# mayuelala/FollowYourClick

Hardware: AMD Instinct MI355X
Metric: denoised frames/sec, 16f x 512^2 clip @ 25 DDIM steps (higher is better)
Workload: dtype bf16; 1 GPU; configs[1]: AnimationPipeline DDIM loop, SD-1.5 UNet3D + mm_sd_v15-shaped motion modules (random init), 1 clip/GPU of 16 frames 512x512, 25 DDIM steps, CFG 8.0, mask + first-frame concat, fps/flow conditioning; frames=16, height=512, width=512, ddim_steps=25, parallelism=dp1 (independent clips, weight broadcast 0.00 GiB in 0.00s)

## Files before the change

### followyourclick_amd/_build.py

```python
import concurrent.futures as cf
import hashlib
import os
import shutil
import subprocess
import sys

HERE = os.path.dirname(os.path.abspath(__file__))
CSRC = os.path.join(HERE, "csrc")
EXTRA = os.environ.get("FYC_BUILD_EXTRA", "").split()
LIB = os.path.abspath(os.environ.get("FYC_BUILD_LIB") or os.path.join(HERE, "libfyc_hip.so"))
OBJ = os.path.join(HERE, "_obj") if not (EXTRA or os.environ.get("FYC_BUILD_LIB")) else LIB + ".obj"
SOURCES = ["api.hip", "gemm.hip", "gemm_bf16_plain.hip", "gemm_bf16_conv.hip", "gemm_bf16_act.hip", "gemm_f16_plain.hip", "gemm_f16_conv.hip", "gemm_f16_act.hip", "gemm_f32.hip", "gemm_bf16_t3.hip", "gemm_f16_t3.hip", "gemm_f32_t3.hip", "gemm_f32x3.hip", "gemm_f32x3_t3.hip", "attention.hip", "attention_small.hip", "attention_medium.hip", "attention_large.hip", "attention_small_f16.hip", "attention_medium_f16.hip", "attention_large_f16.hip", "attention_f32x3.hip", "attention_wide.hip", "attention_wide_f16.hip", "attention_wide_f32x3.hip", "temporal_attn.hip", "temporal_attn_f32x3.hip", "temporal_block.hip", "temporal_block_rr.hip", "ff_block.hip", "panel_linear.hip", "norm.hip", "elementwise.hip"]
FLAGS = ["--offload-arch=gfx950", "-O3", "-std=c++17", "-fPIC", "-ffp-contract=off", "-Wno-unused-value",
         "-mllvm", "-amdgpu-mfma-vgpr-form=1"]
AGPR_SOURCES = {"ff_block.hip", "panel_linear.hip", "temporal_block_rr.hip", "attention_wide.hip", "attention_wide_f16.hip", "attention_wide_f32x3.hip"}


NO_SLP_SOURCES = set(filter(None, os.environ.get("FYC_NO_SLP", "ff_block.hip,gemm_f32x3.hip,gemm_f32x3_t3.hip").split(",")))


NO_NAN_SOURCES = {s for s in SOURCES if s.startswith("attention")}


def _flags(src: str):
    fl = FLAGS
    if src in AGPR_SOURCES:
        fl = [f for f in FLAGS if f not in ("-mllvm", "-amdgpu-mfma-vgpr-form=1")]
    if src in NO_SLP_SOURCES:
        fl = fl + ["-fno-slp-vectorize"]
    if src in NO_NAN_SOURCES and os.environ.get("FYC_ATTN_HONOR_NANS") != "1":
        fl = fl + ["-fno-honor-nans"]
    return fl + EXTRA


def _hipcc() -> str:
    for c in (os.environ.get("HIPCC"), shutil.which("hipcc"), "/opt/rocm/bin/hipcc"):
        if c and os.path.exists(c):
            return c
    raise RuntimeError("hipcc not found (need ROCm with gfx950 support)")


def _digest(path: str) -> str:
    h = hashlib.sha256()
    headers = sorted(os.path.join(CSRC, f) for f in os.listdir(CSRC) if f.endswith(".h"))
    for dep in [path, *headers, os.path.join(HERE, "..", "include", "fyc.h")]:
        with open(dep, "rb") as f:
            h.update(f.read())
    h.update(" ".join(_flags(os.path.basename(path))).encode())
    return h.hexdigest()


def source_digest() -> str:
    h = hashlib.sha256()
    files = sorted(f for f in os.listdir(CSRC) if f.endswith((".hip", ".h")))
    for f in files:
        h.update(f.encode())
        with open(os.path.join(CSRC, f), "rb") as fh:
            h.update(fh.read())
    with open(os.path.join(HERE, "..", "include", "fyc.h"), "rb") as fh:
        h.update(fh.read())
    for src in SOURCES:
        h.update((src + " " + " ".join(_flags(src))).encode())
    return h.hexdigest()


def family_digest(family: str = "gemm") -> str:
    if family != "gemm":
        raise ValueError(family)
    h = hashlib.sha256()
    files = sorted(f for f in os.listdir(CSRC) if f.startswith("gemm") and f.endswith((".hip", ".h"))) + ["fyc_common.h"]
    for f in files:
        h.update(f.encode())
        with open(os.path.join(CSRC, f), "rb") as fh:
            h.update(fh.read())
    for src in SOURCES:
        if src.startswith("gemm"):
            h.update((src + " " + " ".join(_flags(src))).encode())
    return h.hexdigest()


def _compile(src: str) -> str:
    path = os.path.join(CSRC, src)
    obj = os.path.join(OBJ, src.replace(".hip", ".o"))
    stamp = obj + ".sha"
    dig = _digest(path)
    if os.path.exists(obj) and os.path.exists(stamp) and open(stamp).read() == dig:
        return obj
    cmd = [_hipcc(), *_flags(src), "-c", path, "-o", obj]
    r = subprocess.run(cmd, capture_output=True, text=True)
    if r.returncode != 0:
        raise RuntimeError(f"hipcc failed for {src}:\n{r.stderr[-4000:]}")
    with open(stamp, "w") as f:
        f.write(dig)
    return obj

# ... 21 lines not shown
```

### followyourclick_amd/_lib.py

```python
from __future__ import annotations

import ctypes as C
import os

HERE = os.path.dirname(os.path.abspath(__file__))
LIB_PATH = os.environ.get("FYC_LIB_PATH") or os.path.join(HERE, "libfyc_hip.so")

FYC_F32, FYC_BF16, FYC_F16 = 0, 1, 2
GEMM_PLAIN, GEMM_CONV3X3, GEMM_CONV3X3_UP2, GEMM_CONV_T3 = 0, 1, 2, 3
EPI_LINEAR, EPI_GEGLU, EPI_HEADS = 0, 1, 2
ACT_NONE, ACT_GELU, ACT_QUICK_GELU = 0, 1, 2
PRODUCTS_EXACT, PRODUCTS_SPLIT_BF16 = 0, 1

i32, i64, f32, vp = C.c_int32, C.c_int64, C.c_float, C.c_void_p


class GemmArgs(C.Structure):
    _fields_ = [("a", vp), ("a2", vp), ("w", vp), ("bias", vp), ("rowbias", vp), ("residual", vp), ("out", vp),
                ("seg_out", vp * 3), ("seg_transposed", i32 * 3), ("seg_ld", i32 * 3),
                ("M", i32), ("N", i32), ("K", i32),
                ("lda", i32), ("ldw", i32), ("ldo", i32), ("ldr", i32), ("ldrb", i32), ("k_split", i32), ("lda2", i32),
                ("stride_a", i64), ("stride_w", i64), ("stride_o", i64),
                ("batch", i32), ("mode", i32), ("epilogue", i32),
                ("Hout", i32), ("Wout", i32), ("Hin", i32), ("Win", i32), ("Cin", i32), ("conv_stride", i32), ("conv_pad", i32),
                ("rows_per_batch", i32), ("seg_cols", i32), ("heads", i32), ("tokens", i32),
                ("out_scale", f32), ("dtype", i32), ("tile", i32), ("act", i32), ("ln_stats", vp), ("ln_colsum", vp),
                ("ln_nparts", i32), ("ln_eps", f32), ("chan_parts", vp), ("cs_rows", i32), ("row_parts", vp), ("row_nparts", i32), ("workspace", vp), ("workspace_bytes", i64),
                ("t3_frames", i32), ("t3_rows", i32), ("f32_products", i32)]


class AttnArgs(C.Structure):
    _fields_ = [("q", vp), ("k", vp), ("vt", vp), ("o", vp),
                ("batch", i32), ("heads", i32), ("n_q", i32), ("n_k", i32), ("d", i32),
                ("ldo", i32), ("ldvt", i32), ("kv_batch_div", i32), ("o_accumulate", i32),
                ("scale", f32), ("o_scale", f32), ("dtype", i32), ("q_batch_mod", i32), ("f32_products", i32)]


class AttnMaskArgs(C.Structure):
    _fields_ = [("attn", AttnArgs), ("causal", i32)]


class TAttnArgs(C.Structure):
    _fields_ = [("qkv", vp), ("o", vp), ("clips", i32), ("frames", i32), ("pixels", i32), ("heads", i32), ("d", i32),
                ("scale", f32), ("dtype", i32), ("rope_cos", vp), ("rope_sin", vp), ("f32_products", i32)]


class GnStatsArgs(C.Structure):
    _fields_ = [("x", vp), ("stats", vp), ("rows", i32), ("C", i32), ("groups", i32), ("rows_per_sample", i32), ("dtype", i32),
                ("pad_", i32), ("workspace", vp), ("workspace_bytes", i64)]


class GnApplyArgs(C.Structure):
    _fields_ = [("x", vp), ("stats", vp), ("gamma", vp), ("beta", vp), ("y", vp),
                ("rows", i32), ("C", i32), ("groups", i32), ("rows_per_sample", i32), ("eps", f32), ("silu", i32), ("dtype", i32)]


class ChanStatsReduceArgs(C.Structure):
    _fields_ = [("parts", vp), ("cs", vp), ("rows", i32), ("N", i32), ("cs_rows", i32), ("tile_rows", i32), ("slots", i32), ("out_rows", i32)]


class GnApplyCsArgs(C.Structure):
    _fields_ = [("x1", vp), ("cs1", vp), ("x2", vp), ("cs2", vp), ("gamma", vp), ("beta", vp), ("y", vp),
                ("C1", i32), ("C2", i32), ("rows", i32), ("groups", i32), ("rows_per_sample", i32), ("eps", f32), ("silu", i32),
                ("dtype", i32), ("cs_rows", i32), ("parts1", vp), ("parts2", vp),
                ("tile_rows1", i32), ("slots1", i32), ("tile_rows2", i32), ("slots2", i32), ("parts_cs_rows", i32)]


class LayerNormArgs(C.Structure):
    _fields_ = [("x", vp), ("gamma", vp), ("beta", vp), ("pe", vp), ("y", vp),
                ("rows", i32), ("C", i32), ("eps", f32), ("pe_div", i32), ("pe_rows", i32), ("dtype", i32)]


class RowStatsArgs(C.Structure):
    _fields_ = [("x", vp), ("stats", vp), ("rows", i32), ("C", i32), ("eps", f32), ("dtype", i32)]


class SoftmaxArgs(C.Structure):
    _fields_ = [("x", vp), ("rows", i64), ("cols", i32), ("ld", i32), ("dtype", i32), ("causal_rows", i32)]


class ConcatArgs(C.Structure):
    _fields_ = [("a", vp), ("b", vp), ("y", vp), ("rows", i64), ("c1", i32), ("c2", i32), ("dtype", i32)]


class RepeatArgs(C.Structure):
    _fields_ = [("src", vp), ("dst", vp), ("bytes", i64), ("times", i32)]


class SiluArgs(C.Structure):
    _fields_ = [("x", vp), ("y", vp), ("n", i64)]


class CastArgs(C.Structure):
    _fields_ = [("x", vp), ("y", vp), ("rows", i64), ("cols", i32), ("ld", i32), ("dtype", i32)]


class UnetInputArgs(C.Structure):
    _fields_ = [("latents", vp), ("mask", vp), ("first", vp), ("x", vp),
                ("B", i32), ("F", i32), ("HW", i32), ("c_latent", i32), ("c_pad", i32), ("cfg_dup", i32), ("mask_frames", i32),
                ("dtype", i32), ("mode", i32)]


class CfgDdimArgs(C.Structure):
    _fields_ = [("pred", vp), ("latents", vp), ("coef", vp),
                ("B", i32), ("F", i32), ("HW", i32), ("c_latent", i32), ("ld", i32), ("cfg", i32), ("guidance", f32),
                ("pred_type", i32), ("clip_sample", i32), ("dtype", i32), ("pred_single", vp), ("video_scale", f32),
                ("variance_noise", vp), ("sigma", f32), ("clipped_model_output", i32)]


class CfgDdimRescaleArgs(C.Structure):
    _fields_ = [("step", CfgDdimArgs), ("guidance_rescale", f32), ("workspace", vp), ("workspace_bytes", i64)]


class CfgSolverArgs(C.Structure):
    _fields_ = [("pred", vp), ("latents", vp), ("coef", vp),
                ("B", i32), ("F", i32), ("HW", i32), ("c_latent", i32), ("ld", i32), ("cfg", i32), ("guidance", f32),
                ("dtype", i32), ("pred_single", vp), ("video_scale", f32),
                ("hist_out", vp), ("hist_1", vp), ("hist_2", vp), ("order", i32),
                ("guidance_rescale", f32), ("workspace", vp), ("workspace_bytes", i64)]


class NchwInArgs(C.Structure):
    _fields_ = [("z", vp), ("x", vp), ("N", i32), ("C", i32), ("HW", i32), ("c_pad", i32), ("scale", f32), ("dtype", i32)]


class NhwcOutArgs(C.Structure):
    _fields_ = [("x", vp), ("y", vp), ("N", i32), ("C", i32), ("HW", i32), ("ld", i32),
                ("mul", f32), ("add", f32), ("lo", f32), ("hi", f32), ("dtype", i32)]


class EmbedArgs(C.Structure):
    _fields_ = [("ids", vp), ("table", vp), ("pos", vp), ("out", vp), ("rows", i64), ("seq", i32), ("C", i32), ("vocab", i32),
                ("dtype", i32)]


class PatchifyArgs(C.Structure):
    _fields_ = [("image", vp), ("out", vp), ("B", i32), ("Cin", i32), ("H", i32), ("W", i32), ("P", i32), ("ld", i32), ("dtype", i32)]


class TemporalBlockArgs(C.Structure):
    _fields_ = [("x", vp), ("out", vp), ("w_qkv", vp), ("colsum", vp), ("bias", vp), ("pe_bias", vp), ("w_out", vp), ("b_out", vp),
                ("clips", i32), ("frames", i32), ("pixels", i32), ("heads", i32), ("d", i32), ("C", i32),
                ("scale", C.c_float), ("eps", C.c_float), ("dtype", i32), ("wstream", vp)]


class FFBlockArgs(C.Structure):
    _fields_ = [("x", vp), ("residual", vp), ("out", vp), ("wstream", vp), ("b_out", vp), ("chan_parts", vp), ("cs_rows", i32),
                ("rows", i32), ("C", i32), ("hidden", i32), ("eps", C.c_float), ("dtype", i32)]


class PanelLinearArgs(C.Structure):
    _fields_ = [("x", vp), ("residual", vp), ("out", vp), ("wstream", vp), ("bias", vp), ("gn_cs", vp), ("gn_gamma", vp), ("gn_beta", vp),
                ("gn_rows_per_sample", i32), ("gn_stat_samples", i32), ("gn_groups", i32), ("gn_eps", C.c_float),
                ("rows", i32), ("N", i32), ("K", i32), ("dtype", i32), ("gn_parts", vp), ("gn_tile_rows", i32), ("gn_slots", i32)]


class PackConv3x3Args(C.Structure):
    _fields_ = [("w", vp), ("out", vp), ("O", i32), ("I", i32), ("dtype", i32)]


class PackGegluArgs(C.Structure):
    _fields_ = [("w", vp), ("b", vp), ("w_out", vp), ("b_out", vp), ("O", i32), ("I", i32), ("dtype", i32)]


OPS = {
    "fyc_gemm": GemmArgs, "fyc_attention": AttnArgs, "fyc_attention_masked": AttnMaskArgs, "fyc_temporal_attention": TAttnArgs,
    "fyc_gn_stats": GnStatsArgs, "fyc_gn_apply": GnApplyArgs, "fyc_layernorm": LayerNormArgs,
    "fyc_softmax_rows": SoftmaxArgs, "fyc_concat_channels": ConcatArgs, "fyc_silu_f32": SiluArgs,
    "fyc_cast_from_f32": CastArgs, "fyc_cast_to_f32": CastArgs, "fyc_unet_input": UnetInputArgs,
    "fyc_cfg_ddim_step": CfgDdimArgs, "fyc_cfg_ddim_step_rescaled": CfgDdimRescaleArgs, "fyc_cfg_solver_step": CfgSolverArgs, "fyc_nchw_to_nhwc": NchwInArgs, "fyc_nhwc_to_nchw": NhwcOutArgs,
    "fyc_embed_tokens": EmbedArgs, "fyc_patchify": PatchifyArgs, "fyc_row_stats": RowStatsArgs,
    "fyc_gn_apply_cs": GnApplyCsArgs, "fyc_chan_stats_reduce": ChanStatsReduceArgs,
    "fyc_pack_conv3x3": PackConv3x3Args, "fyc_pack_geglu": PackGegluArgs, "fyc_temporal_block": TemporalBlockArgs,
    "fyc_ff_block": FFBlockArgs, "fyc_panel_linear": PanelLinearArgs, "fyc_repeat": RepeatArgs,
}
MISC = ["fyc_version", "fyc_last_error", "fyc_init", "fyc_device_caps", "fyc_set_tuning", "fyc_gemm_row_parts", "fyc_gemm_stat_layout", "fyc_gemm_workspace_bytes", "fyc_gn_stats_workspace", "fyc_temporal_block_supported", "fyc_temporal_block_wstream_bytes",
        "fyc_ff_block_supported", "fyc_ff_block_wstream_bytes", "fyc_panel_linear_supported", "fyc_panel_linear_wstream_bytes",
        "fyc_cfg_ddim_rescale_workspace_bytes", "fyc_cfg_solver_workspace_bytes"]

_lib = None
FYC_VERSION = 308


class FycError(RuntimeError):
    pass


def load() -> C.CDLL:
    global _lib
    if _lib is not None:
        return _lib
    if not os.path.exists(LIB_PATH):
        raise FycError(f"{LIB_PATH} is missing: build it with `python -m followyourclick_amd._build` "
                       "(hipcc --offload-arch=gfx950). There is no CPU fallback.")
    lib = C.CDLL(LIB_PATH)
    lib.fyc_version.restype = C.c_int
    ab_build = bool(os.environ.get("FYC_LIB_PATH"))
    if lib.fyc_version() != FYC_VERSION and not ab_build:
        raise FycError(f"{LIB_PATH} reports ABI version {lib.fyc_version()}, this binding was written against {FYC_VERSION}: argument structs differ "
                       "between major versions - rebuild the library (`python -m followyourclick_amd._build`)")
    lib.fyc_last_error.restype = C.c_char_p
    lib.fyc_init.argtypes = [vp]
    lib.fyc_device_caps.argtypes = [C.POINTER(i64)]
    lib.fyc_set_tuning.argtypes = [C.c_int, C.c_int]
    if not ab_build or hasattr(lib, "fyc_gemm_row_parts"):
        lib.fyc_gemm_row_parts.argtypes = [C.POINTER(GemmArgs)]
        lib.fyc_gemm_row_parts.restype = C.c_int
        lib.fyc_gemm_stat_layout.argtypes = [C.POINTER(GemmArgs), C.POINTER(i32), C.POINTER(i32)]
        lib.fyc_gemm_stat_layout.restype = C.c_int
        lib.fyc_gemm_workspace_bytes.argtypes = [C.POINTER(GemmArgs)]
        lib.fyc_gemm_workspace_bytes.restype = i64
    if not ab_build or hasattr(lib, "fyc_gn_stats_workspace"):
        lib.fyc_gn_stats_workspace.argtypes = [C.POINTER(GnStatsArgs)]
        lib.fyc_gn_stats_workspace.restype = i64
    if not ab_build or hasattr(lib, "fyc_temporal_block_supported"):
        lib.fyc_temporal_block_supported.argtypes = [C.POINTER(TemporalBlockArgs)]
        lib.fyc_temporal_block_supported.restype = C.c_int
    if not ab_build or hasattr(lib, "fyc_temporal_block_wstream_bytes"):
        lib.fyc_temporal_block_wstream_bytes.argtypes = []
        lib.fyc_temporal_block_wstream_bytes.restype = i64
    if not ab_build or hasattr(lib, "fyc_ff_block_supported"):
        lib.fyc_ff_block_supported.argtypes = [C.POINTER(FFBlockArgs)]
        lib.fyc_ff_block_supported.restype = C.c_int
        lib.fyc_ff_block_wstream_bytes.argtypes = []
        lib.fyc_ff_block_wstream_bytes.restype = i64
    if not ab_build or hasattr(lib, "fyc_panel_linear_supported"):
        lib.fyc_panel_linear_supported.argtypes = [C.POINTER(PanelLinearArgs)]
        lib.fyc_panel_linear_supported.restype = C.c_int
        lib.fyc_panel_linear_wstream_bytes.argtypes = [i32, i32]
        lib.fyc_panel_linear_wstream_bytes.restype = i64
    if not ab_build or hasattr(lib, "fyc_cfg_ddim_rescale_workspace_bytes"):
        lib.fyc_cfg_ddim_rescale_workspace_bytes.argtypes = [C.POINTER(CfgDdimRescaleArgs)]
        lib.fyc_cfg_ddim_rescale_workspace_bytes.restype = i64
    if not ab_build or hasattr(lib, "fyc_cfg_solver_workspace_bytes"):
        lib.fyc_cfg_solver_workspace_bytes.argtypes = [C.POINTER(CfgSolverArgs)]
        lib.fyc_cfg_solver_workspace_bytes.restype = i64
    for name, st in OPS.items():
        if ab_build and not hasattr(lib, name):
            continue
        fn = getattr(lib, name)
        fn.argtypes = [C.POINTER(st), vp]
        fn.restype = C.c_int
    _lib = lib
    return lib


def check(rc: int, what: str) -> None:
    if rc != 0:
        raise FycError(f"{what} failed (rc={rc}): {load().fyc_last_error().decode(errors='replace')}")
```

### followyourclick_amd/csrc/gemm_kernel.h

```cpp
#pragma once
#include <mutex>
#include <type_traits>

#include "fyc_common.h"

namespace fycg {

constexpr int FYC_MAX_DEVICES = 64;

struct GemmP {
  const char* a; const char* a2; const char* w; const float* bias; const float* rowbias; const char* residual; char* out;
  char* seg_out[3]; int seg_transposed[3]; int seg_ld[3];
  int M, N, K, lda, ldw, ldo, ldr, ldrb, k_split, lda2;
  long long stride_a, stride_w, stride_o;
  int mode, epilogue;
  int Hout, Wout, Hin, Win, Cin, conv_stride, conv_pad;
  int rows_per_batch, seg_cols, heads, tokens, head_dim;
  float out_scale;
  int act;
  const float* ln_stats; const float* ln_colsum;
  int ln_nparts; float ln_eps;
  float* chan_parts; int cs_rows, cs_slots;
  float* row_parts; int row_nparts;
  int tiles_m, tiles_n;
  int strip;
  int up_exact2; float up_sh, up_sw;
  int colc;
  int rb_tile;
  int rb_slots;
  int splitk; int t3_frames; float* ws;
  int stagger;
  int wide;
  const char* zero;
  int res_acc;
  float inv_seg_cols, inv_head_dim;
  int fast1;
  int heads_pk;
  int pre;
  int phase_delay; int t3_rows;
  unsigned long long* trace;
};
static_assert(sizeof(GemmP) == 392, "GemmP grew: the kernel-argument offsets of every instantiation move");

#ifdef FYC_TRACE
#define FYC_STAMP_DECL int fyc_trace_n = 0
#define FYC_STAMP(p, wave, lane)                                                                                         \
  do {                                                                                                                   \
    if ((p).trace != nullptr && ((wave) & 3) == 0 && (lane) == 0 && fyc_trace_n < 128)                                   \
      (p).trace[((size_t)blockIdx.x * 2 + ((wave) >> 2)) * 128 + fyc_trace_n] = __builtin_amdgcn_s_memtime();            \
    ++fyc_trace_n;                                                                                                       \
  } while (0)
#define FYC_STAMP_E(p, wave, lane, cnt)                                                                                  \
  do {                                                                                                                   \
    if ((p).trace != nullptr && ((wave) & 3) == 0 && (lane) == 0 && (cnt) < 128)                                         \
      (p).trace[65536 + ((size_t)blockIdx.x * 2 + ((wave) >> 2)) * 128 + (cnt)] = __builtin_amdgcn_s_memtime();          \
    ++(cnt);                                                                                                             \
  } while (0)
#else
#define FYC_STAMP_DECL
#define FYC_STAMP(p, wave, lane) do { } while (0)
#define FYC_STAMP_E(p, wave, lane, cnt) do { } while (0)
#endif

__device__ __forceinline__ void tile_coords(const GemmP& p, int t, int& tile_m, int& tile_n) {
  if (p.strip <= 0) { tile_n = t % p.tiles_n; tile_m = t / p.tiles_n; return; }
  const int per_strip = p.strip * p.tiles_m;
  const int s = t / per_strip, r = t - s * per_strip;
  const int n0 = s * p.strip;
  const int w = min(p.strip, p.tiles_n - n0);
  tile_m = r / w;
  tile_n = n0 + r - tile_m * w;
}

template <typename T> struct Mma;
template <> struct Mma<bf16_t> {
  typedef bf16x8 Frag;
  __device__ static __forceinline__ f32x4 mma(Frag a, Frag b, f32x4 c) {
    return __builtin_amdgcn_mfma_f32_16x16x32_bf16(a, b, c, 0, 0, 0);
  }
};
template <> struct Mma<f16_t> {
  typedef f16x8 Frag;
  __device__ static __forceinline__ f32x4 mma(Frag a, Frag b, f32x4 c) {
    return __builtin_amdgcn_mfma_f32_16x16x32_f16(a, b, c, 0, 0, 0);
  }
};
template <> struct Mma<float> {
  typedef f32x4 Frag;
  __device__ static __forceinline__ f32x4 mma(Frag a, Frag b, f32x4 c) {
    c = __builtin_amdgcn_mfma_f32_16x16x4f32(a[0], b[0], c, 0, 0, 0);
    c = __builtin_amdgcn_mfma_f32_16x16x4f32(a[1], b[1], c, 0, 0, 0);
// ... 195 lines not shown
#pragma unroll
  for (int i = 1; i < WTM; ++i) rb_same = rb_same && rbo[i] == rbo[0];
  const bool has_ln = LN && p.ln_stats != nullptr;
  auto pass1_fast = [&](auto ln_c, auto rb_c) __attribute__((always_inline)) {
    constexpr bool HAS_LN = decltype(ln_c)::value, HAS_RB = decltype(rb_c)::value;
    f32x2 rs2[WTM], nm2[WTM];
#pragma unroll
    for (int i = 0; i < WTM; ++i) { rs2[i] = (f32x2){rs[i], rs[i]}; nm2[i] = (f32x2){-rs[i] * mu[i], -rs[i] * mu[i]}; }
    const float* rb0 = HAS_RB ? rbc + rbo[0] : colc;
    f32x4 b4n = *reinterpret_cast<const f32x4*>(colc + nl_w0 + g * 4), s4n = (f32x4){0.f, 0.f, 0.f, 0.f}, r4n = (f32x4){0.f, 0.f, 0.f, 0.f};
    if (HAS_LN) s4n = *reinterpret_cast<const f32x4*>(colc + BN + nl_w0 + g * 4);
    if (HAS_RB) r4n = *reinterpret_cast<const f32x4*>(rb0 + nl_w0 + g * 4);
#pragma unroll
    for (int j = 0; j < WTN; ++j) {
      const int nl = nl_w0 + j * 16 + g * 4;
      f32x4 b4 = b4n;
      const f32x4 s4 = s4n;
      if (HAS_RB) { b4[0] += r4n[0]; b4[1] += r4n[1]; b4[2] += r4n[2]; b4[3] += r4n[3]; }
      __builtin_amdgcn_sched_barrier(0);
      if (j + 1 < WTN) {
        b4n = *reinterpret_cast<const f32x4*>(colc + nl + 16);
        if (HAS_LN) s4n = *reinterpret_cast<const f32x4*>(colc + BN + nl + 16);
        if (HAS_RB) r4n = *reinterpret_cast<const f32x4*>(rb0 + nl + 16);
      }
      const f32x2 b01 = {b4[0], b4[1]}, b23 = {b4[2], b4[3]}, s01 = {s4[0], s4[1]}, s23 = {s4[2], s4[3]};
#pragma unroll
      for (int i = 0; i < WTM; ++i) {
        f32x2 v01 = {acc[i][j][0], acc[i][j][1]}, v23 = {acc[i][j][2], acc[i][j][3]};
        if (HAS_LN) {
          v01 = __builtin_elementwise_fma(v01, rs2[i], __builtin_elementwise_fma(nm2[i], s01, b01));
          v23 = __builtin_elementwise_fma(v23, rs2[i], __builtin_elementwise_fma(nm2[i], s23, b23));
        } else {
          v01 = v01 + b01; v23 = v23 + b23;
        }
        unsigned lo = Pair16<T>::pack(v01[0], v01[1]), hi = Pair16<T>::pack(v23[0], v23[1]);
        asm volatile("" : "+v"(lo), "+v"(hi));
        pk[i][j] = (u32x2){lo, hi};
      }
      __builtin_amdgcn_sched_barrier(0);
    }
  };
  if (p.out_scale == 1.0f && (rbc == nullptr || rb_same) && p.fast1) {
    if (has_ln) { if (rbc != nullptr) pass1_fast(std::true_type{}, std::true_type{}); else pass1_fast(std::true_type{}, std::false_type{}); }
    else { if (rbc != nullptr) pass1_fast(std::false_type{}, std::true_type{}); else pass1_fast(std::false_type{}, std::false_type{}); }
  } else {
  f32x4 b4n = *reinterpret_cast<const f32x4*>(colc + nl_w0 + g * 4), s4n = (f32x4){0.f, 0.f, 0.f, 0.f};
  if (LN && p.ln_stats) s4n = *reinterpret_cast<const f32x4*>(colc + BN + nl_w0 + g * 4);
#pragma unroll
  for (int j = 0; j < WTN; ++j) {
    const int nl = nl_w0 + j * 16 + g * 4;
    const f32x4 b4 = b4n, s4 = s4n;
    __builtin_amdgcn_sched_barrier(0);
    if (j + 1 < WTN) {
      b4n = *reinterpret_cast<const f32x4*>(colc + nl + 16);
      if (LN && p.ln_stats) s4n = *reinterpret_cast<const f32x4*>(colc + BN + nl + 16);
    }
#pragma unroll
    for (int i = 0; i < WTM; ++i) {
      f32x4 v = acc[i][j];
      if (LN && p.ln_stats) {
#pragma unroll
        for (int r = 0; r < 4; ++r) v[r] = rs[i] * (v[r] - mu[i] * s4[r]);
      }
#pragma unroll
      for (int r = 0; r < 4; ++r) v[r] += b4[r];
      if (rbc != nullptr) {
        const f32x4 r4 = *reinterpret_cast<const f32x4*>(rbc + rbo[i] + nl);
#pragma unroll
        for (int r = 0; r < 4; ++r) v[r] += r4[r];
      }
      unsigned lo = Pair16<T>::pack(v[0] * p.out_scale, v[1] * p.out_scale), hi = Pair16<T>::pack(v[2] * p.out_scale, v[3] * p.out_scale);
      asm volatile("" : "+v"(lo), "+v"(hi));
      pk[i][j] = (u32x2){lo, hi};
    }
    __builtin_amdgcn_sched_barrier(0);
  }
  }
  FYC_STAMP_E(p, wave, lane, ecnt);
  const int lrow = lane / CPR, lch = lane - lrow * CPR;
  const bool lact = lrow < RPP;
  const int n_lane = n_w0 + lch * 8;
  const int first_sample = do_cs ? (tile_m * BM) / p.cs_rows : 0;
  const bool one_slot = p.cs_slots == 1;
  float cs8[8], cq8[8];
#pragma unroll
  for (int e = 0; e < 8; ++e) cs8[e] = cq8[e] = 0.f;
  int cur_slot = one_slot ? 0 : -1;
  auto flush_tree = [&](int slot) __attribute__((always_inline)) {
    float* red = reinterpret_cast<float*>(stg);
    float* own = cacc + (wm + slot) * (BN * 2);
    constexpr int NCOL = CPR * 8, ROWS_LIVE = RPP < 16 ? RPP : 16;
#pragma unroll
    for (int ph = 0; ph < 2; ++ph) {
      if (lact) {
        const float* src = ph ? cq8 : cs8;
        *reinterpret_cast<f32x4*>(red + lane * 8) = (f32x4){src[0], src[1], src[2], src[3]};
        *reinterpret_cast<f32x4*>(red + lane * 8 + 4) = (f32x4){src[4], src[5], src[6], src[7]};
      }
      asm volatile("s_waitcnt lgkmcnt(0)" ::: "memory");
#pragma unroll 1
      for (int c = lane; c < NCOL; c += 64) {
        float t = 0.f;
#pragma unroll
        for (int r = 0; r < ROWS_LIVE; ++r) t += red[r * NCOL + c];
        own[(nl_w0 + c) * 2 + ph] = t;
      }
      asm volatile("s_waitcnt lgkmcnt(0)" ::: "memory");
    }
#pragma unroll
    for (int e = 0; e < 8; ++e) cs8[e] = cq8[e] = 0.f;
  };
#pragma unroll
  for (int i = 0; i < WTM; ++i) {
    if (do_cs && !one_slot) {
      const int slot = (tile_m * BM + (wm * WTM + i) * 16) / p.cs_rows - first_sample;
      if (slot != cur_slot) { if (cur_slot >= 0) flush_tree(cur_slot); cur_slot = slot; }
    }
#pragma unroll
    for (int j = 0; j < WTN; ++j) *reinterpret_cast<u32x2*>(stg + r16 * PITCH + j * 32 + g * 8) = pk[i][j];
    asm volatile("s_waitcnt lgkmcnt(0)" ::: "memory");
#pragma unroll
    for (int q = 0; q < NQ; ++q) {
      u32x4 v4q;
      {
        const int rowc = (q * RPP + lrow) < 15 ? (q * RPP + lrow) : 15;
        v4q = *reinterpret_cast<const u32x4*>(stg + rowc * PITCH + lch * 16);
      }
      asm volatile("s_waitcnt lgkmcnt(0)" ::: "memory");
      const int row = q * RPP + lrow;
      const int m = tile_m * BM + (wm * WTM + i) * 16 + row;
      float rsum = 0.f, rsq = 0.f;
      const bool live = lact && row < 16 && m < p.M && n_lane < p.N;
      if (live) {
        const u32x4 v4 = v4q;
        *reinterpret_cast<u32x4*>(O + (long long)m * p.ldo + n_lane) = v4;
        if (do_cs || do_rp) {
#pragma unroll
          for (int e = 0; e < 4; ++e) {
            const float x0 = Pair16<T>::lo(v4[e]), x1 = Pair16<T>::hi(v4[e]);
            if (do_cs) {
              cs8[2 * e] += x0; cq8[2 * e] = __builtin_fmaf(x0, x0, cq8[2 * e]);
              cs8[2 * e + 1] += x1; cq8[2 * e + 1] = __builtin_fmaf(x1, x1, cq8[2 * e + 1]);
            }
            if (do_rp) { rsum += x0 + x1; rsq = __builtin_fmaf(x0, x0, __builtin_fmaf(x1, x1, rsq)); }
          }
        }
      }
      if (do_rp && live) {
        float* dst = racc + ((wm * WTM + i) * 16 + row) * 2;
        lds_add(dst, rsum); lds_add(dst + 1, rsq);
      }
    }
    asm volatile("s_waitcnt lgkmcnt(0)" ::: "memory");
  }
  FYC_STAMP_E(p, wave, lane, ecnt);
  if (do_cs) flush_tree(cur_slot);
  if (do_cs || do_rp) stats_flush<BM, BN, WGM, WGM * WGN * 64>(p, cacc, tile_m, tile_n, wave * 64 + lane);
}

template <typename T, int BM, int BN, int WGM, int WGN, int STG_BYTES, int MODE>
__device__ __forceinline__ void epilogue_heads_packed(const GemmP& p, f32x4 (&acc)[BM / WGM / 16][BN / WGN / 16], int tile_m, int tile_n,
                                                      char* stg_stage, int wave, int lane, const char* pre) {
  static_assert(sizeof(T) == 2, "16-bit outputs only (bf16 / f16)");
  constexpr int WTM = BM / WGM / 16, WTN = BN / WGN / 16;
  constexpr bool LN = (MODE == FYC_GEMM_PLAIN);
  constexpr int PITCH = WTN * 32 + 16, CPR = WTN * 2, RPP = 64 / CPR, NQ = (16 + RPP - 1) / RPP;
  constexpr int SLICE = 16 * PITCH;
  static_assert(WGM * WGN * SLICE + 2 * BN * 4 <= STG_BYTES, "staging + column constants must fit in one ring stage");
  const int wm = wave / WGN, wn = wave % WGN;
  const int g = lane >> 4, r16 = lane & 15;
  __builtin_amdgcn_s_barrier();
  char* stg = stg_stage + wave * SLICE;
  float* colc = reinterpret_cast<float*>(stg_stage + WGM * WGN * SLICE);
  if (pre != nullptr) colc = reinterpret_cast<float*>(const_cast<char*>(pre) + BM * 8);
  else stage_col_constants<BN, LN>(p, colc, tile_m * BM, tile_n, wave * 64 + lane);
  const bool has_ln = LN && p.ln_stats != nullptr;
  f32x2 rs2[WTM], nm2[WTM];
#pragma unroll
  for (int i = 0; i < WTM; ++i) {
    float mu = 0.f, rs = 1.f;
    if (has_ln) {
      if (pre != nullptr) pre_ln_row<BM>(pre, (wm * WTM + i) * 16 + r16, mu, rs);
      else if (tile_m * BM + (wm * WTM + i) * 16 + r16 < p.M) ln_row(p, tile_m * BM + (wm * WTM + i) * 16 + r16, mu, rs);
    }
    rs2[i] = (f32x2){rs * p.out_scale, rs * p.out_scale}; nm2[i] = (f32x2){-rs * mu, -rs * mu};
  }
  const int nl_w0 = wn * WTN * 16, n_w0 = tile_n * BN + nl_w0;
  const f32x2 sc2 = {p.out_scale, p.out_scale};
  u32x2 pk[WTM][WTN];
  auto pass1 = [&](auto ln_c) __attribute__((always_inline)) {
    constexpr bool HAS_LN = decltype(ln_c)::value;
#pragma unroll
    for (int j = 0; j < WTN; ++j) {
      const int nl = nl_w0 + j * 16 + g * 4;
      const f32x4 b4 = *reinterpret_cast<const f32x4*>(colc + nl);
      f32x4 s4 = (f32x4){0.f, 0.f, 0.f, 0.f};
      if (HAS_LN) s4 = *reinterpret_cast<const f32x4*>(colc + BN + nl);
      __builtin_amdgcn_sched_barrier(0);
      const f32x2 b01 = {b4[0], b4[1]}, b23 = {b4[2], b4[3]}, s01 = {s4[0], s4[1]}, s23 = {s4[2], s4[3]};
#pragma unroll
      for (int i = 0; i < WTM; ++i) {
        f32x2 v01 = {acc[i][j][0], acc[i][j][1]}, v23 = {acc[i][j][2], acc[i][j][3]};
        if (HAS_LN) {
          v01 = __builtin_elementwise_fma(v01, rs2[i], sc2 * __builtin_elementwise_fma(nm2[i], s01, b01));
          v23 = __builtin_elementwise_fma(v23, rs2[i], sc2 * __builtin_elementwise_fma(nm2[i], s23, b23));
        } else {
          v01 = (v01 + b01) * sc2; v23 = (v23 + b23) * sc2;
        }
        unsigned lo = Pair16<T>::pack(v01[0], v01[1]), hi = Pair16<T>::pack(v23[0], v23[1]);
        asm volatile("" : "+v"(lo), "+v"(hi));
        pk[i][j] = (u32x2){lo, hi};
      }
      __builtin_amdgcn_sched_barrier(0);
    }
  };
  if (has_ln) pass1(std::true_type{}); else pass1(std::false_type{});
  const int lrow = lane / CPR, lch = lane - lrow * CPR;
  const int n_a = n_w0 + lch * 8;
// ... 114 lines not shown
        unsigned lo = Pair16<T>::pack(lo2.x, lo2.y), hi = Pair16<T>::pack(hi2.x, hi2.y);
        asm volatile("" : "+v"(lo), "+v"(hi));
        pk[i][jo] = (u32x2){lo, hi};
      }
      __builtin_amdgcn_sched_barrier(0);
    }
  };
  if (has_ln) pass1(std::true_type{}); else pass1(std::false_type{});
  const int lrow = lane / CPR, lch = lane - lrow * CPR;
  const bool lact = lrow < RPP;
  const int n_out = p.N >> 1;
  const int n_lane = ((tile_n * BN + nl_w0) >> 1) + lch * 8;
#pragma unroll
  for (int i = 0; i < WTM; ++i) {
#pragma unroll
    for (int jo = 0; jo < OT; ++jo) *reinterpret_cast<u32x2*>(stg + r16 * PITCH + jo * 32 + g * 8) = pk[i][jo];
    asm volatile("s_waitcnt lgkmcnt(0)" ::: "memory");
    u32x4 v4q[NQ];
#pragma unroll
    for (int q = 0; q < NQ; ++q) {
      const int rowc = (q * RPP + lrow) < 15 ? (q * RPP + lrow) : 15;
      v4q[q] = *reinterpret_cast<const u32x4*>(stg + rowc * PITCH + lch * 16);
    }
    asm volatile("s_waitcnt lgkmcnt(0)" ::: "memory");
#pragma unroll
    for (int q = 0; q < NQ; ++q) {
      const int row = q * RPP + lrow;
      const int m = tile_m * BM + (wm * WTM + i) * 16 + row;
      if (lact && row < 16 && m < p.M && n_lane < n_out) *reinterpret_cast<u32x4*>(O + (long long)m * p.ldo + n_lane) = v4q[q];
    }
  }
}

template <typename T, int BM, int BN, int WGM, int WGN>
__device__ __forceinline__ void load_residual_acc(const GemmP& p, f32x4 (&acc)[BM / WGM / 16][BN / WGN / 16], int tile_m, int tile_n, int wave, int lane) {
  constexpr int WTM = BM / WGM / 16, WTN = BN / WGN / 16;
  const int wm = wave / WGN, wn = wave % WGN;
  const int g = lane >> 4, r16 = lane & 15;
  const T* R = reinterpret_cast<const T*>(p.residual);
  const T* zero = reinterpret_cast<const T*>(p.zero);
  constexpr int NP = WTN / 2;
  u32x4 raw16[WTM][NP > 0 ? NP : 1];
  u32x2 raw[WTM][WTN - 2 * NP > 0 ? WTN - 2 * NP : 1];
#pragma unroll
  for (int i = 0; i < WTM; ++i) {
    const int m = tile_m * BM + (wm * WTM + i) * 16 + r16;
#pragma unroll
    for (int jp = 0; jp < NP; ++jp) {
      const int n = tile_n * BN + (wn * WTN + 2 * jp) * 16 + g * 8;
      const T* ptr = (m < p.M && n < p.N) ? R + ((long long)m * p.ldr + n) : zero;
      raw16[i][jp] = *reinterpret_cast<const u32x4*>(ptr);
    }
#pragma unroll
    for (int j = 2 * NP; j < WTN; ++j) {
      const int n = tile_n * BN + (wn * WTN + j) * 16 + g * 4;
      const T* ptr = (m < p.M && n < p.N) ? R + ((long long)m * p.ldr + n) : zero;
      raw[i][j - 2 * NP] = *reinterpret_cast<const u32x2*>(ptr);
    }
  }
  __builtin_amdgcn_sched_barrier(0);
#pragma unroll
  for (int i = 0; i < WTM; ++i) {
#pragma unroll
    for (int jp = 0; jp < NP; ++jp) {
      unsigned x0 = raw16[i][jp][0], x1 = raw16[i][jp][1], y0 = raw16[i][jp][2], y1 = raw16[i][jp][3];
      auto a = __builtin_amdgcn_permlane16_swap(x0, y0, false, false);
      auto b = __builtin_amdgcn_permlane16_swap(x1, y1, false, false);
      auto c = __builtin_amdgcn_permlane32_swap(a[0], a[1], false, false);
      auto d = __builtin_amdgcn_permlane32_swap(b[0], b[1], false, false);
      acc[i][2 * jp] = (f32x4){Pair16<T>::lo(c[0]), Pair16<T>::hi(c[0]), Pair16<T>::lo(d[0]), Pair16<T>::hi(d[0])};
      acc[i][2 * jp + 1] = (f32x4){Pair16<T>::lo(c[1]), Pair16<T>::hi(c[1]), Pair16<T>::lo(d[1]), Pair16<T>::hi(d[1])};
    }
#pragma unroll
    for (int j = 2 * NP; j < WTN; ++j)
      acc[i][j] = (f32x4){Pair16<T>::lo(raw[i][j - 2 * NP][0]), Pair16<T>::hi(raw[i][j - 2 * NP][0]), Pair16<T>::lo(raw[i][j - 2 * NP][1]), Pair16<T>::hi(raw[i][j - 2 * NP][1])};
  }
}

template <typename T, int BM, int BN, int WGM, int WGN, int EPI, int STG_BYTES, int MODE, bool WIDE>
__device__ __forceinline__ void gemm_epilogue(const GemmP& p, f32x4 (&acc)[BM / WGM / 16][BN / WGN / 16], int tile_m, int tile_n,
                                              long long bz, char* stg_stage, int wave, int lane, const char* pre, int& ecnt) {
  constexpr int WTM = BM / WGM / 16, WTN = BN / WGN / 16;
  constexpr bool LN = (MODE == FYC_GEMM_PLAIN);
  const int wm = wave / WGN, wn = wave % WGN;
  const int g = lane >> 4, r16 = lane & 15;
  T* O = reinterpret_cast<T*>(p.out) + bz * p.stride_o;
  const T* R = reinterpret_cast<const T*>(p.residual);
  if constexpr (WIDE && EPI == FYC_EPI_HEADS && sizeof(T) == 2) {
    if (p.fast1 && p.heads_pk) {
      epilogue_heads_packed<T, BM, BN, WGM, WGN, STG_BYTES, MODE>(p, acc, tile_m, tile_n, stg_stage, wave, lane, pre);
      return;
    }
  }
  if constexpr (WIDE && EPI == FYC_EPI_HEADS) {
    constexpr int JG = (WTN + 1) / 2;
    constexpr int PITCH = JG * 64 + 16;
    static_assert(WGM * WGN * 16 * PITCH + 2 * BN * 4 <= STG_BYTES, "staging + column constants must fit in one ring stage");
    __builtin_amdgcn_s_barrier();
    char* stg = stg_stage + wave * (16 * PITCH);
    float* colc = reinterpret_cast<float*>(stg_stage + WGM * WGN * 16 * PITCH);
    if (pre != nullptr) colc = reinterpret_cast<float*>(const_cast<char*>(pre) + BM * 8);
    else stage_col_constants<BN, LN>(p, colc, tile_m * BM, tile_n, wave * 64 + lane);
    const int n_w0 = tile_n * BN + wn * WTN * 16, nl_w0 = wn * WTN * 16;
#pragma unroll
    for (int i = 0; i < WTM; ++i) {
      const int m0 = tile_m * BM + (wm * WTM + i) * 16;
      float ln_mu = 0.f, ln_rs = 1.f;
      if (LN && p.ln_stats) {
        if (pre != nullptr) pre_ln_row<BM>(pre, (wm * WTM + i) * 16 + r16, ln_mu, ln_rs);
        else if (m0 + r16 < p.M) ln_row(p, m0 + r16, ln_mu, ln_rs);
      }
      const int b = m0 / p.tokens, tok0 = m0 - b * p.tokens;
#pragma unroll
      for (int h = 0; h < 2; ++h) {
        const int j0 = h * JG;
        const int nj = (WTN - j0 < JG) ? (WTN - j0) : JG;
        if (nj <= 0) continue;
#pragma unroll
        for (int jj = 0; jj < JG; ++jj) {
          const int jo = j0 + jj;
          if (jo >= WTN) continue;
          const int nl = nl_w0 + jo * 16 + g * 4;
          f32x4 v = acc[i][jo];
          const f32x4 s4 = *reinterpret_cast<const f32x4*>(colc + BN + nl), b4 = *reinterpret_cast<const f32x4*>(colc + nl);
#pragma unroll
          for (int r = 0; r < 4; ++r) v[r] = ((LN && p.ln_stats ? ln_rs * (v[r] - ln_mu * s4[r]) : v[r]) + b4[r]) * p.out_scale;
          *reinterpret_cast<f32x4*>(stg + r16 * PITCH + (jj * 16 + g * 4) * 4) = v;
        }
        asm volatile("s_waitcnt lgkmcnt(0)" ::: "memory");
        const int n0 = n_w0 + j0 * 16;
        if (m0 < p.M) {
          const int cpr = nj * 2;
          for (int c = lane; c < 16 * cpr; c += 64) {
            const int row = c / cpr, ch = c - row * cpr;
            const int n = n0 + ch * 8;
            if (n >= p.N) continue;
            const int seg = fdiv_small(n, p.inv_seg_cols), cs = n - seg * p.seg_cols;
            if (p.seg_transposed[seg]) continue;
            const int hh = fdiv_small(cs, p.inv_head_dim), di = cs - hh * p.head_dim;
            float v8[8];
            *reinterpret_cast<f32x4*>(v8) = *reinterpret_cast<const f32x4*>(stg + row * PITCH + ch * 32);
            *reinterpret_cast<f32x4*>(v8 + 4) = *reinterpret_cast<const f32x4*>(stg + row * PITCH + ch * 32 + 16);
            T* S = reinterpret_cast<T*>(p.seg_out[seg]);
            store8<T>(S + ((long long)(b * p.heads + hh) * p.tokens + tok0 + row) * p.head_dim + di, v8);
          }
          for (int u = lane; u < nj * 32; u += 64) {
            const int col = u >> 1, half = u & 1;
            const int n = n0 + col;
            if (n >= p.N) continue;
            const int seg = fdiv_small(n, p.inv_seg_cols), cs = n - seg * p.seg_cols;
            if (!p.seg_transposed[seg]) continue;
            const int hh = fdiv_small(cs, p.inv_head_dim), di = cs - hh * p.head_dim;
            float v8[8];
#pragma unroll
            for (int r = 0; r < 8; ++r) v8[r] = *reinterpret_cast<const float*>(stg + (half * 8 + r) * PITCH + col * 4);
            T* S = reinterpret_cast<T*>(p.seg_out[seg]);
            store8<T>(S + ((long long)(b * p.heads + hh) * p.head_dim + di) * p.seg_ld[seg] + tok0 + half * 8, v8);
          }
        }
        asm volatile("s_waitcnt lgkmcnt(0)" ::: "memory");
      }
    }
    return;
  }
  if constexpr (WIDE && EPI == FYC_EPI_LINEAR) {
    epilogue_linear_packed<T, BM, BN, WGM, WGN, STG_BYTES, MODE>(p, acc, tile_m, tile_n, bz, stg_stage, wave, lane, pre, ecnt);
// ... 240 lines not shown
        } else {
          const int seg = n / p.seg_cols, c = n - seg * p.seg_cols;
          const int h = c / p.head_dim, di = c - h * p.head_dim;
          const int b = m / p.tokens, tok = m - b * p.tokens;
          T* S = reinterpret_cast<T*>(p.seg_out[seg]);
#pragma unroll
          for (int r = 0; r < 4; ++r) v[r] *= p.out_scale;
          if (!p.seg_transposed[seg]) {
            ElemIO<T>::st4(S + ((long long)(b * p.heads + h) * p.tokens + tok) * p.head_dim + di, v);
          } else {
#pragma unroll
            for (int r = 0; r < 4; ++r)
              ElemIO<T>::st(S + ((long long)(b * p.heads + h) * p.head_dim + di + r) * p.seg_ld[seg] + tok, v[r]);
          }
        }
      }
      if (do_rp) { float* dst = racc + ((wm * WTM + i) * 16 + r16) * 2; lds_add(dst, st_rs); lds_add(dst + 1, st_rq); }
    }
    }
    if constexpr (STATS_OK) {
      if (do_cs) {
        float* own = cacc + (wm + st_slot) * (BN * 2) + ((wn * WTN) * 16 + g * 4) * 2;
#pragma unroll
        for (int j = 0; j < WTN; ++j) {
#pragma unroll
          for (int r = 0; r < 4; ++r) {
            float sx = xs[j][r], sq = xs[j][r] * xs[j][r];
#pragma unroll
            for (int o = 1; o < 16; o <<= 1) { sx += __shfl_xor(sx, o); sq += __shfl_xor(sq, o); }
            if (r16 == 0) { own[(j * 16 + r) * 2] += sx; own[(j * 16 + r) * 2 + 1] += sq; }
          }
        }
      }
    }
  }
  if (do_cs || do_rp) stats_flush<BM, BN, WGM, WGM * WGN * 64>(p, cacc, tile_m, tile_n, wave * 64 + lane);
  }
}

template <int S> using KStep = std::integral_constant<int, S>;
template <typename T, int BM, int BN, int WGM, int WGN, int MODE, int EPI, int NS, int RB = 128, bool WIDE = false, typename P = T>
__global__ void __launch_bounds__(WGM* WGN * 64) fyc_gemm_kernel(const GemmP p) {
  typedef Mma<P> Tr;
  typedef typename Tr::Frag Frag;
  constexpr int NT = WGM * WGN * 64;
  constexpr int CH = 16 / (int)sizeof(T);
  constexpr int CPR = RB / 16;
  constexpr int BK = CPR * CH;
  constexpr int KSTEPS = RB / 64;
  constexpr int A_IT = BM * CPR / NT, B_IT = BN * CPR / NT;
  constexpr int LOADS = A_IT + B_IT;
  constexpr int WTM = BM / WGM / 16, WTN = BN / WGN / 16;
  static_assert(EPI != FYC_EPI_GEGLU || WTN % 2 == 0, "GEGLU pairs value / gate column blocks inside a wave");
  constexpr bool SPLIT3 = std::is_same<P, f32x3_t>::value;
  static_assert(std::is_same<P, T>::value || (SPLIT3 && std::is_same<T, float>::value && RB == 128 && WGM * WGN == 4),
                "f32x3: float storage, one 32-float K tile per matrix instruction, the 4-wave tiles of the f32 mode");
  constexpr int A_BYTES = BM * RB, STAGE = (BM + BN) * RB;
  constexpr bool STAGGER = (WGM * WGN == 8) && KSTEPS >= 2 && NS == 2;
  static_assert(A_IT * NT == BM * CPR && B_IT * NT == BN * CPR, "tile/threads mismatch");
  static_assert(NS >= 2 && NS <= 4 && (NS - 2) * LOADS < 64, "ring depth");
  extern __shared__ __attribute__((aligned(16))) char smem[];

  const int tid = threadIdx.x, lane = tid & 63;
  const int wave = __builtin_amdgcn_readfirstlane(tid >> 6);
  const int wm = wave / WGN, wn = wave % WGN;

  const int ntiles = p.tiles_m * p.tiles_n;
  auto remap = [&](int t) {
    const int q = ntiles >> 3, r = ntiles & 7, xcd = t & 7, idx = t >> 3;
    return (xcd < r ? xcd * (q + 1) : r * (q + 1) + (xcd - r) * q) + idx;
  };
  const long long bz = blockIdx.z;
  const T* __restrict__ A = reinterpret_cast<const T*>(p.a) + bz * p.stride_a;
  const T* __restrict__ W = reinterpret_cast<const T*>(p.w) + bz * p.stride_w;
  const T* __restrict__ A2 = reinterpret_cast<const T*>(p.a2);
  const T* zero = reinterpret_cast<const T*>(p.zero);

  const int lrow = tid / CPR;
  const int koff = ((tid % CPR) ^ swz_key<RB>(lrow)) * CH;
  constexpr int ROWS_IT = NT / CPR;
  static_assert(ROWS_IT % 16 == 0, "row stride per DMA instruction must keep the swizzle key");
  int i_tm = 0, i_tn = 0;
  unsigned a_base = 0, a2_base = 0, b_base = 0;
  constexpr bool C3 = (MODE == FYC_GEMM_CONV3X3);
  constexpr bool T3 = (MODE == FYC_GEMM_CONV_T3);
  constexpr int TAPS = T3 ? 3 : 9;
  static_assert(!T3 || A_IT * 3 <= 32, "CONV_T3: the presence masks of a thread's rows share one register");
  int a_pos[C3 ? A_IT : 1], a_msk[C3 ? A_IT : 1];
  unsigned t_msk = 0, t_step = 0;
  int a_pix[MODE == FYC_GEMM_CONV3X3_UP2 ? A_IT : 1], a_yx[MODE == FYC_GEMM_CONV3X3_UP2 ? A_IT : 1];
  int tap = 0, c0 = 0;
  const int KT = (p.K + BK - 1) / BK;
  const int S = p.splitk > 1 ? p.splitk : 1;
  auto kt_begin = [&](int work) { return (int)(((long long)(work % S) * KT) / S); };
  auto kt_end = [&](int work) { return (int)(((long long)(work % S + 1) * KT) / S); };
  auto setup_issue = [&](int work) {
    const int t = remap(work / S);
    tile_coords(p, t, i_tm, i_tn);
    const int kt0 = kt_begin(work);
    tap = kt0 % TAPS; c0 = (kt0 / TAPS) * BK;
    if (MODE == FYC_GEMM_PLAIN || S == 1) { tap = 0; c0 = 0; }
    b_base = (unsigned)(i_tn * BN + lrow) * (unsigned)p.ldw + koff;
    if (MODE == FYC_GEMM_PLAIN) {
      a_base = (unsigned)(i_tm * BM + lrow) * (unsigned)p.lda + koff;
      a2_base = (unsigned)(i_tm * BM + lrow) * (unsigned)p.lda2 + koff - p.k_split;
    } else if constexpr (T3) {
      a_base = (unsigned)(i_tm * BM + lrow) * (unsigned)p.Cin + koff;
      t_step = (unsigned)p.t3_rows * (unsigned)p.Cin;
      t_msk = 0;
#pragma unroll
      for (int it = 0; it < A_IT; ++it) {
        const int m = i_tm * BM + lrow + it * ROWS_IT;
        const int f = (m / p.t3_rows) % p.t3_frames;
        const unsigned msk = (f > 0 ? 1u : 0u) | 2u | (f + 1 < p.t3_frames ? 4u : 0u);
        if (m < p.M) t_msk |= msk << (3 * it);
      }
    } else {
#pragma unroll
      for (int it = 0; it < A_IT; ++it) {
        const int m = i_tm * BM + lrow + it * ROWS_IT;
        const int hw = p.Hout * p.Wout;
        const int fr = m / hw, rem = m - fr * hw, oy = rem / p.Wout, ox = rem - oy * p.Wout;
        const int iy0 = oy * p.conv_stride - p.conv_pad, ix0 = ox * p.conv_stride - p.conv_pad;
        if (C3) {
          a_pos[it] = fr * p.Hin * p.Win + iy0 * p.Win + ix0;
          int msk = 0;
#pragma unroll
          for (int tp = 0; tp < 9; ++tp) {
            const int iy = iy0 + tp / 3, ix = ix0 + tp % 3;
            if ((unsigned)iy < (unsigned)p.Hin && (unsigned)ix < (unsigned)p.Win) msk |= 1 << tp;
          }
          a_msk[it] = (m < p.M) ? msk : 0;
        } else {
          a_pix[it] = (m < p.M) ? fr * p.Hin * p.Win : -1;
          a_yx[it] = (iy0 << 16) | (ix0 & 0xffff);
        }
      }
    }
  };

  auto src_a = [&](int it, int k0) -> const T* {
    if (MODE == FYC_GEMM_PLAIN) {
      const int m = i_tm * BM + lrow + it * ROWS_IT;
      const int k = k0 + koff;
      if (m >= p.M || k >= p.K) return zero;
      if (A2 != nullptr && k >= p.k_split) return A2 + (size_t)(a2_base + (unsigned)(it * ROWS_IT) * (unsigned)p.lda2 + k0);
      return A + (size_t)(a_base + (unsigned)(it * ROWS_IT) * (unsigned)p.lda + k0);
    } else if constexpr (T3) {
      const unsigned e = a_base + (unsigned)(it * ROWS_IT) * (unsigned)p.Cin + (unsigned)(tap - 1) * t_step + (unsigned)c0;
      return ((t_msk >> (3 * it + tap)) & 1u) ? A + (size_t)e : zero;
    } else if (C3) {
      const int ky = tap / 3, kx = tap - 3 * ky;
      const int pos = a_pos[it] + ky * p.Win + kx;
      return ((a_msk[it] >> tap) & 1) ? A + (size_t)((unsigned)pos * (unsigned)p.Cin + (c0 + koff)) : zero;
    } else {
      const int ky = tap / 3, kx = tap - 3 * ky;
      const int iy = (a_yx[it] >> 16) + ky, ix = (int)(short)(a_yx[it] & 0xffff) + kx;
      const bool ok = a_pix[it] >= 0 && (unsigned)iy < (unsigned)p.Hout && (unsigned)ix < (unsigned)p.Wout;
      int sy, sx;
      if (p.up_exact2) { sy = iy >> 1; sx = ix >> 1; }
      else {
        sy = min((int)floorf((float)iy * p.up_sh), p.Hin - 1);
        sx = min((int)floorf((float)ix * p.up_sw), p.Win - 1);
      }
      return ok ? A + (size_t)((unsigned)(a_pix[it] + sy * p.Win + sx) * (unsigned)p.Cin + c0 + koff) : zero;
    }
  };
  auto src_b = [&](int it, int k0) -> const T* {
    const int n = i_tn * BN + lrow + it * ROWS_IT;
    return (n < p.N && k0 + koff < p.K) ? W + (size_t)(b_base + (unsigned)(it * ROWS_IT) * (unsigned)p.ldw + k0) : zero;
  };

  f32x4 acc[WTM][WTN];
  FYC_STAMP_DECL;
  int fyc_trace_e = 0;

  const int g = lane >> 4, r16 = lane & 15;
  const int sw = swz_key<RB>(r16);
  constexpr bool FRAG_ALL = sizeof(T) == 2 && (WTM * WTN + WTM + WTN) * 4 <= 150;
  constexpr bool FRAG_ROW = sizeof(T) == 2 && !FRAG_ALL;
  constexpr int PF = (WTN >= 8) ? 2 : (WTN >= 4 ? 4 : 6);
  auto compute = [&](int stage, auto first, auto end) {
    constexpr int s0 = decltype(first)::value, s1 = decltype(end)::value;
    const char* sA = smem + stage * STAGE + (wm * WTM * 16 + r16) * RB;
    const char* sB = smem + stage * STAGE + A_BYTES + (wn * WTN * 16 + r16) * RB;
#pragma unroll
    for (int s = 0; s < KSTEPS; ++s) {
      if (s < s0 || s >= s1) continue;
      const int coff = ((4 * s + g) ^ sw) * 16;
      if constexpr (FRAG_ROW) {
        constexpr int RING = PF + 1;
        Frag bfr[WTN], ar[RING];
#pragma unroll
        for (int j = 0; j < WTN; ++j) bfr[j] = *reinterpret_cast<const Frag*>(sB + j * 16 * RB + coff);
#pragma unroll
        for (int i = 0; i < PF && i < WTM; ++i) ar[i % RING] = *reinterpret_cast<const Frag*>(sA + i * 16 * RB + coff);
#pragma unroll
        for (int i = 0; i < WTM; ++i) {
          if (i + PF < WTM) ar[(i + PF) % RING] = *reinterpret_cast<const Frag*>(sA + (i + PF) * 16 * RB + coff);
          __builtin_amdgcn_sched_barrier(0);
#pragma unroll
          for (int j = 0; j < WTN; ++j) acc[i][j] = Tr::mma(bfr[j], ar[i % RING], acc[i][j]);
          __builtin_amdgcn_sched_barrier(0);
        }
        continue;
      }
      Frag af[WTM], bf[WTN];
#pragma unroll
      for (int i = 0; i < WTM; ++i) af[i] = *reinterpret_cast<const Frag*>(sA + i * 16 * RB + coff);
#pragma unroll
      for (int j = 0; j < WTN; ++j) bf[j] = *reinterpret_cast<const Frag*>(sB + j * 16 * RB + coff);
      if (FRAG_ALL) __builtin_amdgcn_sched_barrier(0);
#pragma unroll
      for (int i = 0; i < WTM; ++i)
#pragma unroll
        for (int j = 0; j < WTN; ++j) acc[i][j] = Tr::mma(bf[j], af[i], acc[i][j]);
      if (FRAG_ALL) __builtin_amdgcn_sched_barrier(0);
    }
  };
  constexpr bool XSTEP = FRAG_ALL && KSTEPS == 2 && (WTM * WTN + 2 * (WTM + WTN)) * 4 <= 190;
  auto compute_xstep = [&](int stage, auto&& between) {
    const char* sA = smem + stage * STAGE + (wm * WTM * 16 + r16) * RB;
    const char* sB = smem + stage * STAGE + A_BYTES + (wn * WTN * 16 + r16) * RB;
    const int coff0 = (g ^ sw) * 16, coff1 = ((4 + g) ^ sw) * 16;
    Frag af0[WTM], bf0[WTN], af1[WTM], bf1[WTN];
#pragma unroll
    for (int i = 0; i < WTM; ++i) af0[i] = *reinterpret_cast<const Frag*>(sA + i * 16 * RB + coff0);
#pragma unroll
    for (int j = 0; j < WTN; ++j) bf0[j] = *reinterpret_cast<const Frag*>(sB + j * 16 * RB + coff0);
    __builtin_amdgcn_sched_barrier(0);
#pragma unroll
    for (int i = 0; i < WTM; ++i) af1[i] = *reinterpret_cast<const Frag*>(sA + i * 16 * RB + coff1);
#pragma unroll
    for (int j = 0; j < WTN; ++j) bf1[j] = *reinterpret_cast<const Frag*>(sB + j * 16 * RB + coff1);
    __builtin_amdgcn_sched_barrier(0);
// ... 200 lines not shown
  q.tiles_n = (p.N + BN - 1) / BN;
  q.rb_tile = (p.colc && p.rowbias != nullptr && p.rows_per_batch % BM == 0) ? 1 : 0;
  q.rb_slots = (WIDE && EPI == FYC_EPI_LINEAR && p.rowbias != nullptr && !q.rb_tile) ? rowbias_slots(BM, p.rows_per_batch) : 0;
  {
    constexpr int BK = (RB / 16) * (16 / (int)sizeof(T));
    const int kt = (p.K + BK - 1) / BK;
    const bool rb_ok = p.rowbias == nullptr || (EPI == FYC_EPI_LINEAR && (q.rb_tile || q.rb_slots > 0));
    q.pre = (PRE_BUILT && g_fyc_tuning[FYC_TUNE_NO_PRESTAGE] != 1 && kt >= 2 && !(q.splitk > 1) && p.ln_nparts == 0 && rb_ok && p.wide &&
             (p.ln_stats == nullptr || (p.M % 2 == 0 && ((uintptr_t)p.ln_stats % 16) == 0))) ? 1 : 0;
  }
  q.fast1 = g_fyc_tuning[FYC_TUNE_GENERIC_PASS1] == 1 ? 0 : 1;
  q.heads_pk = g_fyc_tuning[FYC_TUNE_HEADS_PACKED] == 1 ? 1 : g_fyc_tuning[FYC_TUNE_HEADS_PACKED] == 2 ? 0 : (p.M <= 8192 ? 1 : 0);
  q.stagger = g_fyc_tuning[FYC_TUNE_NO_STAGGER] == 1 ? 0 : 1;
  q.phase_delay = g_fyc_tuning[FYC_TUNE_PHASE_DELAY] > 0 ? g_fyc_tuning[FYC_TUNE_PHASE_DELAY] : 0;
  q.res_acc = (WIDE && EPI == FYC_EPI_LINEAR && p.residual != nullptr && p.ln_stats == nullptr && !(q.splitk > 1)) ? 1 : 0;
#ifdef FYC_TRACE
  q.trace = g_fyc_trace;
#endif
  q.strip = (q.tiles_n > 4 && g_fyc_tuning[FYC_TUNE_GEMM_STRIP] >= 0) ? (g_fyc_tuning[FYC_TUNE_GEMM_STRIP] > 0 ? g_fyc_tuning[FYC_TUNE_GEMM_STRIP] : (q.tiles_n >= 16 ? 8 : 4)) : 0;
  int occ = (160 * 1024) / smem;
  const int wave_cap = 32 / (WGM * WGN);
  if (occ > wave_cap) occ = wave_cap;
  if (occ < 1) occ = 1;
  long long resident = (long long)n_cu * occ / (batch > 0 ? batch : 1);
  if (resident < n_cu) resident = n_cu;
  const long long ntiles = (long long)q.tiles_m * q.tiles_n * (q.splitk > 1 ? q.splitk : 1);
  dim3 grid((unsigned)(ntiles < resident ? ntiles : resident), 1, batch);
  hipLaunchKernelGGL(kern, grid, dim3(WGM * WGN * 64), smem, st, q);
  FYC_CHECK_LAUNCH("fyc_gemm");
  return 0;
}

template <typename T, int MODE, int EPI, bool WIDE, typename P = T>
int dispatch_cfg(int cfg, int ns, const GemmP& p, int batch, hipStream_t st) {
  if constexpr (!WIDE) {
    if (cfg != 1 && cfg != 2) cfg = (p.N % 128 == 0 || p.N > 512) ? 1 : 2;
    if (cfg == 1) return launch<T, 128, 128, 2, 2, MODE, EPI, 2, 128, false, P>(p, batch, st);
    return launch<T, 128, 64, 2, 2, MODE, EPI, 2, 128, false, P>(p, batch, st);
  } else {
    switch (cfg) {
      case 1: if (ns == 3) return launch<T, 128, 128, 2, 2, MODE, EPI, 3, 128, true>(p, batch, st);
              return launch<T, 128, 128, 2, 2, MODE, EPI, 2, 128, true>(p, batch, st);
      case 2: if constexpr (MODE == FYC_GEMM_PLAIN) {
                if (ns == 4) return launch<T, 128, 64, 2, 2, MODE, EPI, 4, 128, true>(p, batch, st);
                if (ns == 3) return launch<T, 128, 64, 2, 2, MODE, EPI, 3, 128, true>(p, batch, st);
              }
              return launch<T, 128, 64, 2, 2, MODE, EPI, 2, 128, true>(p, batch, st);
      case 3: return launch<T, 256, 128, 4, 2, MODE, EPI, 2, 128, true>(p, batch, st);
      case 4: return launch<T, 256, 64, 4, 1, MODE, EPI, 2, 128, true>(p, batch, st);
      case 5: return launch<T, 256, 320, 4, 2, MODE, EPI, 2, 128, true>(p, batch, st);
      case 6: if constexpr (EPI == FYC_EPI_GEGLU) FYC_FAIL(-2, "fyc_gemm: tile config 6 gives a wave an odd number of column blocks: not built for GEGLU");
              else return launch<T, 128, 320, 2, 4, MODE, EPI, 2, 128, true>(p, batch, st);
      case 7: return launch<T, 256, 256, 2, 4, MODE, EPI, 2, 128, true>(p, batch, st);
      case 8: return launch<T, 128, 320, 2, 2, MODE, EPI, 2, 64, true>(p, batch, st);
      case 10: return launch<T, 128, 128, 2, 2, MODE, EPI, 2, 64, true>(p, batch, st);
      case 11: if constexpr (EPI == FYC_EPI_GEGLU) FYC_FAIL(-2, "fyc_gemm: tile config 11 gives a wave an odd number of column blocks: not built for GEGLU");
               else return launch<T, 128, 160, 2, 2, MODE, EPI, 2, 128, true>(p, batch, st);
    }
    FYC_FAIL(-2, "fyc_gemm: tile config %d not built", cfg);
  }
}

template <typename T, int MODE, int EPI>
int dispatch_ns(int ns, int cfg, const GemmP& p, int batch, hipStream_t st) {
  if constexpr (sizeof(T) == 2) {
    if (p.wide) return dispatch_cfg<T, MODE, EPI, true>(cfg, ns, p, batch, st);
  }
  return dispatch_cfg<T, MODE, EPI, false>(cfg, ns, p, batch, st);
}

int run_bf16_plain(const GemmP& p, int batch, int cfg, int ns, hipStream_t st);
int run_bf16_conv(const GemmP& p, int batch, int cfg, int ns, hipStream_t st);
int run_bf16_act(const GemmP& p, int batch, int cfg, hipStream_t st);
int run_f32(const GemmP& p, int batch, int cfg, hipStream_t st);
constexpr int CFG_F32X3 = 0x100;
int run_f32x3(const GemmP& p, int batch, int cfg, hipStream_t st);
int run_f32x3_t3(const GemmP& p, int batch, int cfg, hipStream_t st);
int run_f16_plain(const GemmP& p, int batch, int cfg, int ns, hipStream_t st);
int run_f16_conv(const GemmP& p, int batch, int cfg, int ns, hipStream_t st);
int run_f16_act(const GemmP& p, int batch, int cfg, hipStream_t st);
int run_bf16_t3(const GemmP& p, int batch, int cfg, int ns, hipStream_t st);
int run_f16_t3(const GemmP& p, int batch, int cfg, int ns, hipStream_t st);
int run_f32_t3(const GemmP& p, int batch, int cfg, hipStream_t st);

}
```

### followyourclick_amd/engine/base.py

```python
from __future__ import annotations

import os
from typing import Optional, Sequence, Tuple

import torch

from .. import _lib as L

Tensor = torch.Tensor

ALLOC_FILL = int(os.environ["FYC_ALLOC_FILL"]) if os.environ.get("FYC_ALLOC_FILL") else None


def empty(*shape, dtype, device) -> Tensor:
    t = torch.empty(*shape, dtype=dtype, device=device)
    if ALLOC_FILL is not None and t.numel():
        t.view(torch.uint8).fill_(ALLOC_FILL)
    return t


def conv_out_size(Hin: int, Win: int, stride: int = 1, pad: int = 1, up2: bool = False, up_size=None) -> Tuple[int, int]:
    if up2:
        return up_size if up_size is not None else (2 * Hin, 2 * Win)
    return (Hin + pad - 2) // stride + 1, (Win + pad - 2) // stride + 1
# ... 21 lines not shown
    sw = os.environ.get("FYC_SIDE_FLASH", "1")
    if sw == "0":
        return False
    if dtype == torch.float32 and getattr(ops, "f32_products", "exact") != "split":
        return False
    can_causal, max_d = getattr(ops, "attention_causal_supported", None), getattr(ops, "attention_max_head_dim", None)
    if can_causal is None or max_d is None or d % 8 or d > max_d() or (d > 160 and d % 32) or (causal and not can_causal()):
        return False
    return sw == "force" or SIDE_FLASH_DEFAULT[family, _DT_WORD[dtype]]


class EngineBase:
    fuse_stats = True
    direct_stats = False

    def new(self, *shape, dtype=None) -> Tensor:
        return empty(*shape, dtype=dtype or self.dtype, device=self.device)

    def zeros(self, *shape, dtype=None) -> Tensor:
        return torch.zeros(*shape, dtype=dtype or self.dtype, device=self.device)

    def _cs_plan(self, rows: int, stat_rows: int, N: int, K: int, mode: int, out_rows: int) -> Optional[ChanStats]:
        if not self.fuse_stats or stat_rows % 16 or rows % stat_rows:
            return None
        if getattr(self.ops, "abi_version", L.FYC_VERSION) < 301 and self.ops.gemm_split_bytes(self.dtype, M=rows, N=N, K=K, mode=mode) > 0:
            return None
        nt, tile_rows, slots = self.ops.gemm_stat_layout(self.dtype, M=rows, N=N, K=K, cs_rows=stat_rows, mode=mode)
        if not 1 <= slots <= 4:
            return None
        return ChanStats(N, out_rows, parts=self.new(nt * slots * N * 2, dtype=torch.float32), tile_rows=tile_rows, slots=slots, rows=rows,
                         stat_rows=stat_rows)

    def _produced(self, st: Optional[ChanStats]) -> Optional[ChanStats]:
        if st is not None and not self.direct_stats:
            self._stats(st)
        return st

    def _stats(self, st: ChanStats) -> Tensor:
        if st.cs is None:
            st.cs = self.new(st.rows // st.out_rows, st.C, 2, dtype=torch.float64)
            self.ops.chan_stats_reduce(st.parts, st.cs, rows=st.rows, N=st.C, cs_rows=st.stat_rows, tile_rows=st.tile_rows, slots=st.slots,
                                       out_rows=st.out_rows)
        return st.cs

    def _direct_limit(self) -> int:
        return 0

    def _direct(self, sts: Sequence[ChanStats], rows_per_sample: int) -> Optional[int]:
        if not self.direct_stats or any(st.parts is None or st.cs is not None for st in sts):
            return None
        srows = sts[0].stat_rows
        if any(st.stat_rows != srows for st in sts) or rows_per_sample % srows:
            return None
        nbytes = 0
        for st in sts:
            tiles = rows_per_sample // st.tile_rows if rows_per_sample % st.tile_rows == 0 else (rows_per_sample - 1) // st.tile_rows + 2
            nbytes += max(tiles, 1) * st.slots * st.C * 8
        return nbytes if nbytes <= self._direct_limit() else None

    def gn_from_stats(self, srcs: Sequence[Tuple[Tensor, Optional[ChanStats]]], gamma: Tensor, beta: Tensor, rows: int,
                      rows_per_sample: int, eps: float, silu: bool, groups: Optional[int] = None) -> Optional[Tensor]:
        sts = [st for _, st in srcs]
        if any(st is None or st.out_rows != sts[0].out_rows for st in sts) or rows_per_sample % sts[0].out_rows:
            return None
        s1 = sts[0]
        kw = {}
        if len(srcs) == 2:
            kw.update(x2=srcs[1][0], C2=sts[1].C)
        if self._direct(sts, rows_per_sample) is not None:
            cs1 = None
            kw.update(parts1=s1.parts, tile_rows1=s1.tile_rows, slots1=s1.slots, parts_cs_rows=s1.stat_rows)
            if len(srcs) == 2:
                kw.update(parts2=sts[1].parts, tile_rows2=sts[1].tile_rows, slots2=sts[1].slots)
        else:
            cs1 = self._stats(s1)
            if len(srcs) == 2:
                kw.update(cs2=self._stats(sts[1]))
            kw.update(cs_rows=s1.out_rows)
        y = self.new(rows, sum(st.C for st in sts))
        self.ops.gn_apply_cs(srcs[0][0], cs1, gamma, beta, y, rows=rows, C1=s1.C, groups=groups or self.groups, rows_per_sample=rows_per_sample,
                             eps=eps, silu=silu, **kw)
        return y

    def conv_stats(self, x: Tensor, w: Tensor, b: Tensor, frames: int, Hin: int, Win: int, nxt=None, per_frame: bool = False,
                   stride: int = 1, pad: int = 1, up2: bool = False, up_size=None, **kw) -> Tuple[Tensor, Optional[ChanStats]]:
        Cout, K = w.shape
        Ho, Wo = conv_out_size(Hin, Win, stride, pad, up2, up_size)
        if per_frame:
            nxt = (Ho * Wo, Ho * Wo)
        st = None
        if nxt is not None:
            st = self._cs_plan(frames * Ho * Wo, nxt[0], Cout, K, L.GEMM_CONV3X3_UP2 if up2 else L.GEMM_CONV3X3, nxt[1])
        out = self.conv(x, w, b, frames, Hin, Win, stride=stride, pad=pad, up2=up2, up_size=up_size, stats=st, **kw)
        return out, self._produced(st)

    def lin(self, x: Tensor, w: Tensor, rows: int, bias=None, residual=None, geglu=False, out=None) -> Tensor:
        N, K = w.shape
        cols = N // 2 if geglu else N
        out = out if out is not None else self.new(rows, cols, dtype=x.dtype)
        self.ops.gemm(x, w, out, M=rows, N=N, K=K, lda=K, ldw=K, ldo=cols, bias=bias, residual=residual, ldr=cols,
                      epilogue=L.EPI_GEGLU if geglu else L.EPI_LINEAR)
        return out

    def conv(self, x: Tensor, w: Tensor, b: Tensor, frames: int, Hin: int, Win: int, stride: int = 1, up2: bool = False,
             rowbias=None, rpb: int = 1, residual=None, ldrb: int = 0, up_size=None, pad: int = 1, stats: Optional[ChanStats] = None) -> Tensor:
        Cout, K = w.shape
        Cin = K // 9
        Ho, Wo = conv_out_size(Hin, Win, stride, pad, up2, up_size)
        M = frames * Ho * Wo
        out = self.new(M, Cout)
        self.ops.gemm(x, w, out, M=M, N=Cout, K=K, lda=Cin, ldw=K, ldo=Cout, bias=b, rowbias=rowbias, rows_per_batch=rpb, ldrb=ldrb,
                      residual=residual, ldr=Cout, mode=L.GEMM_CONV3X3_UP2 if up2 else L.GEMM_CONV3X3,
                      conv=dict(Hout=Ho, Wout=Wo, Hin=Hin, Win=Win, Cin=Cin, stride=stride, pad=pad),
                      chan_parts=None if stats is None else stats.parts, cs_rows=0 if stats is None else stats.stat_rows)
        return out

    def group_norm(self, x: Tensor, g: Tensor, b: Tensor, rows: int, C: int, rows_per_sample: int, eps: float, silu: bool,
                   groups: Optional[int] = None) -> Tensor:
        groups = groups or self.groups
        stats = self.new(rows // rows_per_sample, groups, 2, dtype=torch.float64)
        self.ops.gn_stats(x, stats, rows=rows, C_=C, groups=groups, rows_per_sample=rows_per_sample)
        y = self.new(rows, C)
        self.ops.gn_apply(x, stats, g, b, y, rows=rows, C_=C, groups=groups, rows_per_sample=rows_per_sample,
                          eps=eps, silu=silu)
        return y

    def layer_norm(self, x: Tensor, gb, rows: int, C: int, pe=None, pe_div: int = 1, pe_rows: int = 1) -> Tensor:
        y = self.new(rows, C)
        self.ops.layernorm(x, gb[0], gb[1], y, rows=rows, C_=C, eps=1e-5, pe=pe, pe_div=pe_div, pe_rows=pe_rows)
        return y
```

### followyourclick_amd/engine/unet3d.py

```python
from __future__ import annotations

import math
import os
from typing import List, Optional, Sequence, Tuple, Union

import torch

from .. import _lib as L
from .. import ops as ops_mod
from .base import ChanStats, EngineBase
from .config import UNet3DConfig
from .weights import Packed, pack_ff_block, pack_panel_linear, pack_temporal_block, rope_tables

Tensor = torch.Tensor

FUSE_STATS = os.environ.get("FYC_FUSE_STATS", "1") != "0"
FUSE_TEMPORAL = os.environ.get("FYC_FUSE_TEMPORAL", "1") != "0"
TEMPORAL_RR = os.environ.get("FYC_TEMPORAL_RR", "1") != "0"
FUSE_FF = os.environ.get("FYC_FUSE_FF", "1") != "0"
FUSE_PANEL = os.environ.get("FYC_FUSE_PANEL", "1") != "0"
PANEL_ALL = os.environ.get("FYC_PANEL_ALL", "0") != "0"
CFG_SHARE = os.environ.get("FYC_CFG_SHARE", "1") != "0"
DIRECT_STATS = os.environ.get("FYC_DIRECT_STATS", "0") != "0"
DIRECT_STATS_BYTES = int(os.environ.get("FYC_DIRECT_STATS_BYTES", str(24 << 10)))
# ... 386 lines not shown
        l0 = self.P.down[0].layers[0] if self.P.down and self.P.down[0].layers else None
        o = self.ops
        return bool(CFG_SHARE and B % 2 == 0 and temb_first is None and l0 is not None and l0.attn is not None and not self.fuse_rows
                    and hasattr(o, "repeat") and hasattr(o, "attention_q_batch_mod_supported") and o.attention_q_batch_mod_supported())

    def forward(self, x: Tensor, temb: Tensor, B: int, F: int, H: int, W: int, temb_first: Optional[Tensor] = None,
                shared_prefix: int = 1) -> Tensor:
        assert self.ctx_cache is not None, "call prepare_context() first"
        cfg, P = self.cfg, self.P
        if shared_prefix not in (1, 2):
            raise ValueError(f"shared_prefix must be 1 or 2, got {shared_prefix}")
        share = shared_prefix == 2 and self.shares_prefix(B, temb_first)
        if shared_prefix == 2 and not share:
            if B % 2:
                raise ValueError(f"shared_prefix=2 needs an even batch, got {B}")
            x = torch.cat([x, x])
        self.last_schedule = "shared" if share else "plain"
        g = dict(B=B, F=F, H=H, W=W, rows=B * F * H * W)
        if temb_first is not None:
            temb = temb.repeat_interleave(F, dim=0)
            temb[0::F] = temb_first
            g["temb_per_frame"] = True
        frames = B * F

        def hw(gg):
            return gg["H"] * gg["W"]

        def frame(gg):
            return hw(gg), hw(gg)

        def clip(gg):
            return hw(gg), (hw(gg) if cfg.use_inflated_groupnorm else F * hw(gg))

        def layer(l, xin, gg):
            y = self.resnet(l.resnet, xin, temb, gg, frame(gg) if (l.attn is not None or l.motion is not None) else clip(gg))
            if l.attn is not None:
                y = self.transformer(l.attn, y, gg, frame(gg) if l.motion is not None else clip(gg))
            if l.motion is not None:
                y = self.motion(l.motion, y, gg, clip(gg))
            return y

        first = None
        if share:
            first = P.down[0].layers[0]
            gh = dict(g, B=B // 2, rows=g["rows"] // 2)
            x = self._conv_act(x, P.conv_in_w, P.conv_in_b, frames // 2, H, W, clip(g))
            skip = self._repeat(x.t, 2)
            skips = [Act(skip, x.C, ChanStats(x.C, x.st.out_rows, cs=self._repeat(self._stats(x.st), 2)) if x.st is not None else None)]
            x = self.resnet(first.resnet, x, temb[:B // 2], gh, frame(g))
            x = self.transformer(first.attn, x, g, frame(g) if first.motion is not None else clip(g), share=2)
            if first.motion is not None:
                x = self.motion(first.motion, x, g, clip(g))
            skips.append(x)
        else:
            x = self._conv_act(x, P.conv_in_w, P.conv_in_b, frames, H, W, clip(g))
            skips = [x]
        sizes = [(H, W)]
        for blk in P.down:
            for l in blk.layers:
                if l is first:
                    continue
                x = layer(l, x, g)
                skips.append(x)
            if blk.down is not None:
                g2 = dict(g, H=(g["H"] - 1) // 2 + 1, W=(g["W"] - 1) // 2 + 1)
                g2["rows"] = B * F * g2["H"] * g2["W"]
                x = self._conv_act(x.t, blk.down.w, blk.down.b, frames, g["H"], g["W"], clip(g2), stride=2)
                g = g2
                sizes.append((g["H"], g["W"]))
                skips.append(x)
        x = self.resnet(P.mid.r0, x, temb, g, frame(g))
        x = self.transformer(P.mid.attn, x, g, frame(g) if P.mid.motion is not None else clip(g))
        if P.mid.motion is not None:
            x = self.motion(P.mid.motion, x, g, clip(g))
        x = self.resnet(P.mid.r1, x, temb, g, clip(g))
        for blk in P.up:
            for l in blk.layers:
                x = layer(l, (x, skips.pop()), g)
            if blk.up is not None:
                sizes.pop()
                Hn, Wn = sizes[-1]
                g2 = dict(g, H=Hn, W=Wn)
                g2["rows"] = B * F * Hn * Wn
                x = self._conv_act(x.t, blk.up.w, blk.up.b, frames, g["H"], g["W"], clip(g2), up2=True, up_size=(Hn, Wn))
                g = g2
        h, _ = self._gn(x, P.out_g, P.out_b, g["rows"], clip(g)[1], cfg.norm_eps, True)
        return self.conv(h, P.conv_out_w, P.conv_out_b, frames, g["H"], g["W"])
```

### followyourclick_amd/engine/vae.py

```python
from __future__ import annotations

import os

import torch

from .. import _lib as L
from .. import ops as ops_mod
from .base import EngineBase, side_flash
from .config import VAEDecoderConfig
from .weights import Packed, pad_channels

FUSE_STATS = os.environ.get("FYC_VAE_FUSE_STATS", "1") != "0"

Tensor = torch.Tensor


class VAEDecoderEngine(EngineBase):
    def __init__(self, packed: Packed, ops=None):
        self.P = packed
        self.cfg: VAEDecoderConfig = packed.cfg
        self.dtype = packed.dtype
        self.ops = ops if ops is not None else ops_mod.get()
        self.device = packed.conv_in_w.device
        self.groups = self.cfg.norm_num_groups
        self.ops.ensure_init(self.device)

    def conv_cs(self, x: Tensor, w: Tensor, b: Tensor, frames: int, Hin: int, Win: int, **kw):
        return self.conv_stats(x, w, b, frames, Hin, Win, per_frame=FUSE_STATS, **kw)

    def gn(self, x: Tensor, cs, g: Tensor, b: Tensor, rows: int, C: int, hw: int, silu: bool) -> Tensor:
        y = self.gn_from_stats([(x, cs)], g, b, rows, hw, 1e-6, silu)
        return y if y is not None else self.group_norm(x, g, b, rows, C, hw, 1e-6, silu)

    def resnet(self, r: Packed, x: Tensor, frames: int, H: int, W: int, cs=None):
        rows, hw = frames * H * W, H * W
        h = self.gn(x, cs, r.n1_g, r.n1_b, rows, r.cin, hw, True)
        h, cs1 = self.conv_cs(h, r.c1_w, r.c1_b, frames, H, W)
        h = self.gn(h, cs1, r.n2_g, r.n2_b, rows, r.cout, hw, True)
        sc = self.lin(x, r.sc_w, rows, bias=r.sc_b) if r.sc_w is not None else x
        return self.conv_cs(h, r.c2_w, r.c2_b, frames, H, W, residual=sc)

    def attention(self, a: Packed, x: Tensor, frames: int, H: int, W: int, cs=None) -> Tensor:
        o = self.ops
        rows, N = frames * H * W, H * W
        C = a.o_w.shape[0]
        h = self.gn(x, cs, a.g, a.b, rows, C, N, False)
        ld = ((N + 7) // 8) * 8
        q, k = self.new(frames, 1, N, C), self.new(frames, 1, N, C)
        vt = self.zeros(frames, 1, C, ld) if ld != N else self.new(frames, 1, C, ld)
        o.gemm(h, a.qkv_w, None, M=rows, N=3 * C, K=C, lda=C, ldw=C, bias=a.qkv_b, epilogue=L.EPI_HEADS,
               heads=dict(seg_cols=C, heads=1, tokens=N, outs=[q, k, vt], transposed=[0, 0, 1], ld=[0, 0, ld]))
        if side_flash(o, h.dtype, "vae", C):
            att = self.new(rows, C)
            o.attention(q, k, vt, att, batch=frames, heads=1, n_q=N, n_k=N, d=C, ldo=C, ldvt=ld, scale=C ** -0.5)
            return self.lin(att, a.o_w, rows, bias=a.o_b, residual=x)
        S = self.zeros(frames, N, ld) if ld != N else self.new(frames, N, ld)
        o.gemm(q, k, S, M=N, N=N, K=C, lda=C, ldw=C, ldo=ld, batch=frames, stride_a=N * C, stride_w=N * C, stride_o=N * ld,
               out_scale=C ** -0.5)
        o.softmax_rows(S, rows=frames * N, cols=N, ld=ld)
        att = self.new(rows, C)
        o.gemm(S, vt, att, M=N, N=C, K=ld, lda=ld, ldw=ld, ldo=C, batch=frames, stride_a=N * ld, stride_w=C * ld, stride_o=N * C)
        return self.lin(att, a.o_w, rows, bias=a.o_b, residual=x)

    def decode(self, z: Tensor, raw: bool = False) -> Tensor:
        P, cfg, o = self.P, self.cfg, self.ops
        N, Cz, H, W = z.shape
        z = z.to(device=self.device, dtype=torch.float32).contiguous()
        cp = pad_channels(Cz)
        x = self.new(N * H * W, cp)
        o.nchw_to_nhwc(z, x, N=N, C_=Cz, HW=H * W, c_pad=cp, scale=1.0 / cfg.scaling_factor)
        y = self.zeros(N * H * W, cp)
        o.gemm(x, P.pq_w, y, M=N * H * W, N=Cz, K=cp, lda=cp, ldw=cp, ldo=cp, bias=P.pq_b)
        x, cs = self.conv_cs(y, P.conv_in_w, P.conv_in_b, N, H, W)
        x, cs = self.resnet(P.mid_r0, x, N, H, W, cs)
        x = self.attention(P.attn, x, N, H, W, cs)
        x, cs = self.resnet(P.mid_r1, x, N, H, W)
        for blk in P.ups:
            for r in blk.resnets:
                x, cs = self.resnet(r, x, N, H, W, cs)
            if blk.up is not None:
                x, cs = self.conv_cs(x, blk.up.w, blk.up.b, N, H, W, up2=True)
                H, W = 2 * H, 2 * W
        c0 = cfg.block_out_channels[0]
        h = self.gn(x, cs, P.out_g, P.out_b, N * H * W, c0, H * W, True)
        Co = cfg.out_channels
        ldo = ((Co + 3) // 4) * 4
        img = self.new(N * H * W, ldo)
        Kc = P.conv_out_w.shape[1]
        o.gemm(h, P.conv_out_w, img, M=N * H * W, N=Co, K=Kc, lda=Kc // 9, ldw=Kc, ldo=ldo, bias=P.conv_out_b, mode=L.GEMM_CONV3X3,
               conv=dict(Hout=H, Wout=W, Hin=H, Win=W, Cin=Kc // 9, stride=1))
        out = self.new(N, Co, H, W, dtype=torch.float32)
        if raw:
            o.nhwc_to_nchw(img, out, N=N, C_=Co, HW=H * W, ld=ldo)
        else:
            o.nhwc_to_nchw(img, out, N=N, C_=Co, HW=H * W, ld=ldo, mul=0.5, add=0.5, lo=0.0, hi=1.0)
        return out

    def decode_video(self, latents: Tensor, chunk: int = 16) -> Tensor:
        B, C, F, H, W = latents.shape
        z = latents.to(self.device, torch.float32).permute(0, 2, 1, 3, 4).reshape(B * F, C, H, W).contiguous()
        outs = [self.decode(z[i:i + chunk]) for i in range(0, B * F, chunk)]
        vid = torch.cat(outs, 0) if len(outs) > 1 else outs[0]
        return vid.reshape(B, F, vid.shape[1], vid.shape[2], vid.shape[3]).permute(0, 2, 1, 3, 4)


class VAEEncoderEngine(VAEDecoderEngine):

    def encode_moments(self, x: Tensor) -> Tensor:
        P, cfg, o = self.P, self.cfg, self.ops
        N, Ci, H, W = x.shape
        x = x.to(device=self.device, dtype=torch.float32).contiguous()
        cp = pad_channels(Ci)
        h = self.new(N * H * W, cp)
        o.nchw_to_nhwc(x, h, N=N, C_=Ci, HW=H * W, c_pad=cp, scale=1.0)
        h, cs = self.conv_cs(h, P.conv_in_w, P.conv_in_b, N, H, W)
        for blk in P.downs:
            for r in blk.resnets:
                h, cs = self.resnet(r, h, N, H, W, cs)
            if blk.down is not None:
                h, cs = self.conv_cs(h, blk.down.w, blk.down.b, N, H, W, stride=2, pad=0)
                H, W = H // 2, W // 2
        h, cs = self.resnet(P.mid_r0, h, N, H, W, cs)
        h = self.attention(P.attn, h, N, H, W, cs)
        h, cs = self.resnet(P.mid_r1, h, N, H, W)
        c = cfg.block_out_channels[-1]
        h = self.gn(h, cs, P.out_g, P.out_b, N * H * W, c, H * W, True)
        C2 = 2 * cfg.latent_channels
        cp2 = pad_channels(C2)
        z = self.zeros(N * H * W, cp2)
        Kc = P.conv_out_w.shape[1]
        o.gemm(h, P.conv_out_w, z, M=N * H * W, N=C2, K=Kc, lda=Kc // 9, ldw=Kc, ldo=cp2, bias=P.conv_out_b, mode=L.GEMM_CONV3X3,
               conv=dict(Hout=H, Wout=W, Hin=H, Win=W, Cin=Kc // 9, stride=1, pad=1))
        m = self.new(N * H * W, 8 if C2 <= 8 else cp2)
        o.gemm(z, P.q_w, m, M=N * H * W, N=C2, K=cp2, lda=cp2, ldw=cp2, ldo=m.shape[1], bias=P.q_b)
        out = self.new(N, C2, H, W, dtype=torch.float32)
        o.nhwc_to_nchw(m, out, N=N, C_=C2, HW=H * W, ld=m.shape[1])
        return out
```

### followyourclick_amd/engine/weights.py

```python
from __future__ import annotations

import os

from typing import Dict, Optional, Tuple

import torch

from .config import UNet3DConfig, VAEDecoderConfig

Tensor = torch.Tensor
K_ALIGN = 64


def pad_channels(c: int) -> int:
    return ((c + K_ALIGN - 1) // K_ALIGN) * K_ALIGN


def conv_slab(dtype) -> int:
    return 128 // torch.empty((), dtype=dtype).element_size()


def pack_conv3x3(w: Tensor, dtype, device) -> Tensor:
    O, I, kh, kw = w.shape
    assert kh == 3 and kw == 3
    Ip, sl = pad_channels(I), conv_slab(dtype)
    p = torch.zeros(O, Ip, 3, 3, dtype=torch.float32)
    p[:, :I] = w
    p = p.reshape(O, Ip // sl, sl, 3, 3).permute(0, 1, 3, 4, 2)
    return p.reshape(O, 9 * Ip).to(dtype).contiguous().to(device)


def pack_conv_t3(w: Tensor, dtype, device) -> Tensor:
    O, I, kt, kh, kw = w.shape
    assert (kt, kh, kw) == (3, 1, 1) and I % K_ALIGN == 0
    sl = conv_slab(dtype)
    p = w.detach().float().reshape(O, I // sl, sl, 3).permute(0, 1, 3, 2)
    return p.reshape(O, 3 * I).to(dtype).contiguous().to(device)


def pack_linear(w: Tensor, dtype, device, k_pad: Optional[int] = None) -> Tensor:
    w = w.reshape(w.shape[0], -1)
    if k_pad is not None and k_pad != w.shape[1]:
        p = torch.zeros(w.shape[0], k_pad, dtype=torch.float32)
        p[:, : w.shape[1]] = w
        w = p
    return w.to(dtype).contiguous().to(device)


def pack_geglu(w: Tensor, b: Tensor, dtype, device):
    O, I = w.shape
    half = O // 2
    assert half % 16 == 0
    wv, wg = w[:half].reshape(half // 16, 16, I), w[half:].reshape(half // 16, 16, I)
    bv, bg = b[:half].reshape(half // 16, 16), b[half:].reshape(half // 16, 16)
    wp = torch.stack([wv, wg], dim=1).reshape(O, I)
    bp = torch.stack([bv, bg], dim=1).reshape(O)
    return wp.to(dtype).contiguous().to(device), bp.float().contiguous().to(device)


def f32(t: Tensor, device) -> Tensor:
    return t.detach().float().contiguous().to(device)


def fold_layernorm(w: Tensor, b: Optional[Tensor], gamma: Tensor, beta: Tensor, dtype, device, geglu: bool = False):
    w = w.reshape(w.shape[0], -1).double()
    wf = (w * gamma.double()[None, :]).float()
    bias = (w @ beta.double() + (b.double() if b is not None else 0.0)).float()
    if geglu:
        wp, bp = pack_geglu(wf, bias, dtype, device)
    else:
        wp, bp = pack_linear(wf, dtype, device), f32(bias, device)
    return wp, bp, wp.float().sum(dim=1).contiguous()

LN_FOLD = os.environ.get("FYC_LN_FOLD", "1") != "0"


class Packed(dict):
    __getattr__ = dict.__getitem__


def _resnet(sd: Dict[str, Tensor], p: str, dtype, device, temb: bool = True) -> Packed:
    r = Packed(
        n1_g=f32(sd[p + ".norm1.weight"], device), n1_b=f32(sd[p + ".norm1.bias"], device),
        c1_w=pack_conv3x3(sd[p + ".conv1.weight"], dtype, device), c1_b=f32(sd[p + ".conv1.bias"], device),
        n2_g=f32(sd[p + ".norm2.weight"], device), n2_b=f32(sd[p + ".norm2.bias"], device),
        c2_w=pack_conv3x3(sd[p + ".conv2.weight"], dtype, device), c2_b=f32(sd[p + ".conv2.bias"], device),
        cin=sd[p + ".conv1.weight"].shape[1], cout=sd[p + ".conv1.weight"].shape[0], sc_w=None, sc_b=None)
    if (p + ".conv_shortcut.weight") in sd:
        r["sc_w"] = pack_linear(sd[p + ".conv_shortcut.weight"], dtype, device)
        r["sc_b"] = f32(sd[p + ".conv_shortcut.bias"], device)
    r["tconv"] = None
    if (p + ".temporal_conv.conv1.0.weight") in sd:
        r["tconv"] = []
        for i in range(1, 5):
            n, c = f"{p}.temporal_conv.conv{i}.0", f"{p}.temporal_conv.conv{i}.{2 if i == 1 else 3}"
            r["tconv"].append(Packed(g=f32(sd[n + ".weight"], device), b=f32(sd[n + ".bias"], device),
                                     w=pack_conv_t3(sd[c + ".weight"], dtype, device), cb=f32(sd[c + ".bias"], device)))
    return r


def _ff(sd, p, dtype, device, proj_out_w: Tensor, proj_out_b: Tensor, ln: Optional[str] = None) -> Packed:
    cs1 = None
    if ln is not None and LN_FOLD:
        w1, b1, cs1 = fold_layernorm(sd[p + ".net.0.proj.weight"], sd[p + ".net.0.proj.bias"], sd[ln + ".weight"], sd[ln + ".bias"],
                                     dtype, device, geglu=True)
    else:
        w1, b1 = pack_geglu(sd[p + ".net.0.proj.weight"], sd[p + ".net.0.proj.bias"], dtype, device)
    w2, b2 = sd[p + ".net.2.weight"].double(), sd[p + ".net.2.bias"].double()
    wp, bp = proj_out_w.reshape(proj_out_w.shape[0], -1).double(), proj_out_b.double()
    merged_w = torch.cat([wp, wp @ w2], dim=1).float()
    merged_b = (bp + wp @ b2).float()
    return Packed(w1=w1, b1=b1, cs1=cs1, po_w=pack_linear(merged_w, dtype, device), po_b=f32(merged_b, device))
# ... 187 lines not shown
    assert N % pn == 0 and pn % 16 == 0 and K % 64 == 0
    fr = _mfma_fragments(w.reshape(N // pn, pn // 16, 16, K // 64, 2, 32).permute(0, 3, 4, 1, 2, 5))
    return fr.reshape(-1).contiguous()


def sinusoidal_pe(channels: int, length: int) -> Tensor:
    import math
    pos = torch.arange(length, dtype=torch.float32)[:, None]
    div = torch.exp(torch.arange(0, channels, 2, dtype=torch.float32) * (-math.log(10000.0) / channels))
    pe = torch.zeros(length, channels)
    pe[:, 0::2] = torch.sin(pos * div)
    pe[:, 1::2] = torch.cos(pos * div)
    return pe.contiguous()


def rope_inv_freq(d: int, base: float = 10000.0) -> Tensor:
    return 1.0 / (base ** (torch.arange(0, d, 2).float() / d))


def rope_tables(d: int, frames: int) -> Tuple[Tensor, Tensor]:
    ang = torch.einsum("i,j->ij", torch.arange(frames, dtype=torch.float32), rope_inv_freq(d))
    return ang.cos().contiguous(), ang.sin().contiguous()


def pack_unet(sd: Dict[str, Tensor], cfg: UNet3DConfig, dtype, device) -> Packed:
    cfg.validate()
    sd = {k: v.detach().float().cpu() for k, v in sd.items()}
    nb = len(cfg.block_out_channels)
    P = Packed(cfg=cfg, dtype=dtype)
    half = 0.5 if cfg.use_first_frame_condition_concat else 1.0
    P["conv_in_w"] = pack_conv3x3(sd["conv_in.weight"] * half, dtype, device)
    P["conv_in_b"] = f32(sd["conv_in.bias"] * half, device)
    emb = {}
    for name in (["time_embedding"] + (["camera_motion_embedding"] if cfg.use_camera_motion_condition else [])
                 + (["fps_embedding", "motion_embedding"] if cfg.use_fps_condition else [])):
        emb[name] = Packed(w1=f32(sd[name + ".linear_1.weight"], device), b1=f32(sd[name + ".linear_1.bias"], device),
                           w2=f32(sd[name + ".linear_2.weight"], device), b2=f32(sd[name + ".linear_2.bias"], device))
    P["emb"] = emb
    resnets, temb_w, temb_b = [], [], []

    def add_resnet(p):
        r = _resnet(sd, p, dtype, device)
        if not cfg.use_temporal_conv:
            r["tconv"] = None
        elif r.tconv is None:
            raise KeyError(f"use_temporal_conv: the state dict has no {p}.temporal_conv.* entries")
        r["temb_off"] = sum(w.shape[0] for w in temb_w)
        temb_w.append(sd[p + ".time_emb_proj.weight"])
        temb_b.append(sd[p + ".time_emb_proj.bias"])
        resnets.append(r)
        return r

    down = []
    for i, bt in enumerate(cfg.down_block_types):
        p = f"down_blocks.{i}"
        layers = []
        for j in range(cfg.layers_per_block):
            layers.append(Packed(
                resnet=add_resnet(f"{p}.resnets.{j}"),
                attn=_transformer(sd, f"{p}.attentions.{j}", cfg, dtype, device, cfg.down_heads(i)) if bt.startswith("CrossAttn") else None,
                motion=_motion(sd, f"{p}.motion_modules.{j}", cfg, dtype, device)
                if cfg.use_motion_module and (2 ** i) in cfg.motion_module_resolutions else None))
        ds = None
        if i != nb - 1:
            ds = Packed(w=pack_conv3x3(sd[f"{p}.downsamplers.0.conv.weight"], dtype, device), b=f32(sd[f"{p}.downsamplers.0.conv.bias"], device))
        down.append(Packed(layers=layers, down=ds))
    P["down"] = down
    P["mid"] = Packed(r0=add_resnet("mid_block.resnets.0"), attn=_transformer(sd, "mid_block.attentions.0", cfg, dtype, device, cfg.mid_heads()),
                      motion=_motion(sd, "mid_block.motion_modules.0", cfg, dtype, device)
                      if cfg.use_motion_module and cfg.motion_module_mid_block else None,
                      r1=add_resnet("mid_block.resnets.1"))
    up = []
    for i, bt in enumerate(cfg.up_block_types):
        p = f"up_blocks.{i}"
        layers = []
        for j in range(cfg.layers_per_block + 1):
            layers.append(Packed(
                resnet=add_resnet(f"{p}.resnets.{j}"),
                attn=_transformer(sd, f"{p}.attentions.{j}", cfg, dtype, device, cfg.up_heads(i)) if bt.startswith("CrossAttn") else None,
                motion=_motion(sd, f"{p}.motion_modules.{j}", cfg, dtype, device)
                if cfg.use_motion_module and (2 ** (nb - 1 - i)) in cfg.motion_module_resolutions else None))
        us = None
        if i != nb - 1:
            us = Packed(w=pack_conv3x3(sd[f"{p}.upsamplers.0.conv.weight"], dtype, device), b=f32(sd[f"{p}.upsamplers.0.conv.bias"], device))
        up.append(Packed(layers=layers, up=us))
    P["up"] = up
    P["out_g"], P["out_b"] = f32(sd["conv_norm_out.weight"], device), f32(sd["conv_norm_out.bias"], device)
    P["conv_out_w"] = pack_conv3x3(sd["conv_out.weight"], dtype, device)
    P["conv_out_b"] = f32(sd["conv_out.bias"], device)
    P["temb_w"] = f32(torch.cat(temb_w, 0), device)
    P["temb_b"] = f32(torch.cat(temb_b, 0), device)
    P["temb_total"] = P["temb_w"].shape[0]
    return P


def pack_vae_decoder(sd: Dict[str, Tensor], cfg: VAEDecoderConfig, dtype, device) -> Packed:
    sd = {k: v.detach().float().cpu() for k, v in sd.items()}
    P = Packed(cfg=cfg, dtype=dtype)
    P["pq_w"] = pack_linear(sd["post_quant_conv.weight"], dtype, device, k_pad=pad_channels(cfg.latent_channels))
    P["pq_b"] = f32(sd["post_quant_conv.bias"], device)
    P["conv_in_w"] = pack_conv3x3(sd["decoder.conv_in.weight"], dtype, device)
    P["conv_in_b"] = f32(sd["decoder.conv_in.bias"], device)
    P["mid_r0"] = _resnet(sd, "decoder.mid_block.resnets.0", dtype, device)
    a = "decoder.mid_block.attentions.0"
    P["attn"] = Packed(g=f32(sd[a + ".group_norm.weight"], device), b=f32(sd[a + ".group_norm.bias"], device),
                       qkv_w=pack_linear(torch.cat([sd[a + ".query.weight"], sd[a + ".key.weight"], sd[a + ".value.weight"]], 0), dtype, device),
                       qkv_b=f32(torch.cat([sd[a + ".query.bias"], sd[a + ".key.bias"], sd[a + ".value.bias"]], 0), device),
                       o_w=pack_linear(sd[a + ".proj_attn.weight"], dtype, device), o_b=f32(sd[a + ".proj_attn.bias"], device))
    P["mid_r1"] = _resnet(sd, "decoder.mid_block.resnets.1", dtype, device)
    ups = []
    nb = len(cfg.block_out_channels)
    for i in range(nb):
        rs = [_resnet(sd, f"decoder.up_blocks.{i}.resnets.{j}", dtype, device) for j in range(cfg.layers_per_block + 1)]
        us = None
        if i != nb - 1:
            k = f"decoder.up_blocks.{i}.upsamplers.0.conv"
            us = Packed(w=pack_conv3x3(sd[k + ".weight"], dtype, device), b=f32(sd[k + ".bias"], device))
        ups.append(Packed(resnets=rs, up=us))
    P["ups"] = ups
    P["out_g"], P["out_b"] = f32(sd["decoder.conv_norm_out.weight"], device), f32(sd["decoder.conv_norm_out.bias"], device)
    P["conv_out_w"] = pack_conv3x3(sd["decoder.conv_out.weight"], dtype, device)
    P["conv_out_b"] = f32(sd["decoder.conv_out.bias"], device)
    return P


def _vae_attn(sd, a: str, dtype, device) -> Packed:
    return Packed(g=f32(sd[a + ".group_norm.weight"], device), b=f32(sd[a + ".group_norm.bias"], device),
                  qkv_w=pack_linear(torch.cat([sd[a + ".query.weight"], sd[a + ".key.weight"], sd[a + ".value.weight"]], 0), dtype, device),
                  qkv_b=f32(torch.cat([sd[a + ".query.bias"], sd[a + ".key.bias"], sd[a + ".value.bias"]], 0), device),
                  o_w=pack_linear(sd[a + ".proj_attn.weight"], dtype, device), o_b=f32(sd[a + ".proj_attn.bias"], device))


def pack_vae_encoder(sd: Dict[str, Tensor], cfg: VAEDecoderConfig, dtype, device) -> Packed:
    sd = {k: v.detach().float().cpu() for k, v in sd.items()}
    P = Packed(cfg=cfg, dtype=dtype)
    P["conv_in_w"] = pack_conv3x3(sd["encoder.conv_in.weight"], dtype, device)
    P["conv_in_b"] = f32(sd["encoder.conv_in.bias"], device)
    downs = []
    nb = len(cfg.block_out_channels)
    for i in range(nb):
        rs = [_resnet(sd, f"encoder.down_blocks.{i}.resnets.{j}", dtype, device) for j in range(cfg.layers_per_block)]
        ds = None
        if i != nb - 1:
            k = f"encoder.down_blocks.{i}.downsamplers.0.conv"
            ds = Packed(w=pack_conv3x3(sd[k + ".weight"], dtype, device), b=f32(sd[k + ".bias"], device))
        downs.append(Packed(resnets=rs, down=ds))
    P["downs"] = downs
    P["mid_r0"] = _resnet(sd, "encoder.mid_block.resnets.0", dtype, device)
    P["attn"] = _vae_attn(sd, "encoder.mid_block.attentions.0", dtype, device)
    P["mid_r1"] = _resnet(sd, "encoder.mid_block.resnets.1", dtype, device)
    P["out_g"], P["out_b"] = f32(sd["encoder.conv_norm_out.weight"], device), f32(sd["encoder.conv_norm_out.bias"], device)
    P["conv_out_w"] = pack_conv3x3(sd["encoder.conv_out.weight"], dtype, device)
    P["conv_out_b"] = f32(sd["encoder.conv_out.bias"], device)
    C2 = 2 * cfg.latent_channels
    P["q_w"] = pack_linear(sd["quant_conv.weight"], dtype, device, k_pad=pad_channels(C2))
    P["q_b"] = f32(sd["quant_conv.bias"], device)
    return P
```

### followyourclick_amd/ops.py

```python
from __future__ import annotations

import os

import ctypes as C
from typing import Optional, Tuple

import torch

from . import _lib as L
from . import default_f32_products

Tensor = torch.Tensor


_DTYPE_CODES = {torch.bfloat16: L.FYC_BF16, torch.float16: L.FYC_F16, torch.float32: L.FYC_F32}


_PRODUCTS = {"exact": L.PRODUCTS_EXACT, "split": L.PRODUCTS_SPLIT_BF16}


def resolve_f32_products(op: str, dtype: torch.dtype, products: Optional[str], instance_mode: str, *, fused_exact: bool = True) -> int:
    if products is not None and products not in _PRODUCTS:
        raise ValueError(f"{op}: products {products!r}: expected None, 'exact' or 'split'")
    if dtype != torch.float32:
# ... 80 lines not shown

    def set_f32_products(self, mode: str) -> None:
        if mode not in _PRODUCTS:
            raise ValueError(f"f32 products {mode!r}: expected 'exact' or 'split'")
        self.f32_products = mode
        self._ws_need.clear()
        self._q_cache.clear()

    def _stream(self) -> int:
        return _raw_stream(self._inited_dev if self._inited_dev is not None else torch.cuda.current_device())

    def _call(self, name: str, args) -> None:
        L.check(getattr(self.lib, name)(C.byref(args), self._stream()), name)

    def gemm(self, a: Tensor, w: Tensor, out: Optional[Tensor], *, M: int, N: int, K: int, lda: int, ldw: int,
             ldo: int = 0, bias: Optional[Tensor] = None, rowbias: Optional[Tensor] = None, rows_per_batch: int = 1,
             residual: Optional[Tensor] = None, ldr: int = 0, ldrb: int = 0, out_scale: float = 1.0, epilogue: int = L.EPI_LINEAR,
             mode: int = L.GEMM_PLAIN, conv: Optional[dict] = None, batch: int = 1, stride_a: int = 0,
             stride_w: int = 0, stride_o: int = 0, heads: Optional[dict] = None, tile: int = 0,
             a2: Optional[Tensor] = None, k_split: int = 0, lda2: int = 0, act: int = L.ACT_NONE,
             ln_stats: Optional[Tensor] = None, ln_colsum: Optional[Tensor] = None, ln_nparts: int = 0, ln_eps: float = 1e-5,
             chan_parts: Optional[Tensor] = None, cs_rows: int = 0, row_parts: Optional[Tensor] = None, row_nparts: int = 0,
             products: Optional[str] = None) -> None:
        self.ensure_init(a.device)
        f32_products = resolve_f32_products("gemm", a.dtype, products, self.f32_products)
        g = self._gemm_args(a, w, out, M=M, N=N, K=K, lda=lda, ldw=ldw, ldo=ldo, bias=bias, rowbias=rowbias, rows_per_batch=rows_per_batch,
                            residual=residual, ldr=ldr, ldrb=ldrb, out_scale=out_scale, epilogue=epilogue, mode=mode, conv=conv, batch=batch,
                            stride_a=stride_a, stride_w=stride_w, stride_o=stride_o, heads=heads, tile=tile, a2=a2, k_split=k_split,
                            lda2=lda2, act=act, ln_stats=ln_stats, ln_colsum=ln_colsum, ln_nparts=ln_nparts, ln_eps=ln_eps,
                            chan_parts=chan_parts, cs_rows=cs_rows, row_parts=row_parts, row_nparts=row_nparts)
        g.f32_products = f32_products
        key = (M, N, K, mode, epilogue, act, batch, tile, g.dtype, ln_stats is not None, chan_parts is not None, row_parts is not None)
        need = self._ws_need.get(key)
        if need is None:
            need = int(self.lib.fyc_gemm_workspace_bytes(C.byref(g))) if hasattr(self.lib, "fyc_gemm_workspace_bytes") else 0
            self._ws_need[key] = need
        if need > 0:
            if self._ws is None or self._ws.numel() < need or self._ws.device != a.device:
                self._ws = torch.empty(need, dtype=torch.uint8, device=a.device)
            g.workspace, g.workspace_bytes = self._ws.data_ptr(), self._ws.numel()
        self._call("fyc_gemm", g)

    def gemm_row_parts(self, dtype: torch.dtype, *, M: int, N: int, K: int, mode: int = L.GEMM_PLAIN, batch: int = 1, tile: int = 0) -> int:
        key = ("rp", dtype, M, N, K, mode, batch, tile)
        if key not in self._q_cache:
            g = L.GemmArgs()
            g.M, g.N, g.K, g.mode, g.batch, g.tile = M, N, K, mode, batch, tile
            g.dtype = _dtc(dtype)
            self._q_cache[key] = int(self.lib.fyc_gemm_row_parts(C.byref(g))) if hasattr(self.lib, "fyc_gemm_row_parts") else 0
        return self._q_cache[key]

    def gemm_split_bytes(self, dtype: torch.dtype, *, M: int, N: int, K: int, mode: int = L.GEMM_PLAIN) -> int:
        key = ("sb", dtype, M, N, K, mode)
        if key not in self._q_cache:
            g = L.GemmArgs()
            g.M, g.N, g.K, g.mode, g.batch, g.epilogue = M, N, K, mode, 1, L.EPI_LINEAR
            g.dtype = _dtc(dtype)
            self._q_cache[key] = int(self.lib.fyc_gemm_workspace_bytes(C.byref(g))) if hasattr(self.lib, "fyc_gemm_workspace_bytes") else 0
        return self._q_cache[key]

    def gemm_stat_layout(self, dtype: torch.dtype, *, M: int, N: int, K: int, cs_rows: int, mode: int = L.GEMM_PLAIN, batch: int = 1,
                         tile: int = 0):
        key = ("sl", dtype, M, N, K, cs_rows, mode, batch, tile)
        if key not in self._q_cache:
            if not hasattr(self.lib, "fyc_gemm_stat_layout"):
                self._q_cache[key] = (0, 0, 0)
            else:
                g = L.GemmArgs()
                g.M, g.N, g.K, g.mode, g.batch, g.tile, g.cs_rows = M, N, K, mode, batch, tile, cs_rows
                g.dtype = _dtc(dtype)
                tr, sl = L.i32(0), L.i32(0)
                n = int(self.lib.fyc_gemm_stat_layout(C.byref(g), C.byref(tr), C.byref(sl)))
                self._q_cache[key] = (n, int(tr.value), int(sl.value))
        return self._q_cache[key]

    def chan_stats_reduce(self, parts: Tensor, cs: Tensor, *, rows: int, N: int, cs_rows: int, tile_rows: int, slots: int,
                          out_rows: int = 0) -> None:
        if cs.dtype != torch.float64:
            raise TypeError("channel statistics must be float64")
        a = L.ChanStatsReduceArgs()
        a.parts, a.cs, a.rows, a.N, a.cs_rows, a.tile_rows, a.slots = _f32(parts, "parts"), _p(cs), rows, N, cs_rows, tile_rows, slots
        a.out_rows = out_rows
        self._call("fyc_chan_stats_reduce", a)

    @staticmethod
    def _gemm_args(a, w, out, *, M, N, K, lda, ldw, ldo, bias, rowbias, rows_per_batch, residual, ldr, ldrb, out_scale, epilogue, mode,
                   conv, batch, stride_a, stride_w, stride_o, heads, tile, a2, k_split, lda2, act, ln_stats, ln_colsum, ln_nparts,
                   ln_eps, chan_parts, cs_rows, row_parts, row_nparts):
        g = L.GemmArgs()
        g.a, g.w, g.bias, g.rowbias = _p(a), _p(w), _f32(bias, "bias"), _f32(rowbias, "rowbias")
        g.residual, g.out = _p(residual), _p(out)
        g.M, g.N, g.K, g.lda, g.ldw, g.ldo, g.ldr, g.ldrb = M, N, K, lda, ldw, ldo, ldr, ldrb
        g.stride_a, g.stride_w, g.stride_o, g.batch = stride_a, stride_w, stride_o, batch
        g.mode, g.epilogue, g.rows_per_batch, g.out_scale, g.dtype = mode, epilogue, rows_per_batch, out_scale, _dt(a)
        g.tile, g.act = tile, act
        g.ln_stats, g.ln_colsum = _f32(ln_stats, "ln_stats"), _f32(ln_colsum, "ln_colsum")
        g.a2, g.k_split, g.lda2 = _p(a2), k_split, lda2
        if a.dtype != w.dtype:
            raise TypeError(f"gemm: activation {a.dtype} vs weight {w.dtype}")
        if conv is not None and mode == L.GEMM_CONV_T3:
            g.Cin, g.t3_frames, g.t3_rows = conv["Cin"], conv["frames"], conv["rows"]
        elif conv is not None:
            g.Hout, g.Wout, g.Hin, g.Win, g.Cin, g.conv_stride = (conv["Hout"], conv["Wout"], conv["Hin"], conv["Win"],
                                                                  conv["Cin"], conv.get("stride", 1))
            g.conv_pad = conv.get("pad", 1)
        if heads is not None:
            g.seg_cols, g.heads, g.tokens = heads["seg_cols"], heads["heads"], heads["tokens"]
            for i, (t, tr, ld) in enumerate(zip(heads["outs"], heads["transposed"], heads["ld"])):
                g.seg_out[i], g.seg_transposed[i], g.seg_ld[i] = _p(t), int(tr), int(ld)
        g.ln_nparts, g.ln_eps = ln_nparts, ln_eps
        g.chan_parts, g.cs_rows = _f32(chan_parts, "chan_parts"), cs_rows
        g.row_parts, g.row_nparts = _f32(row_parts, "row_parts"), row_nparts
        return g

    def attention(self, q: Tensor, k: Tensor, vt: Tensor, o: Tensor, *, batch: int, heads: int, n_q: int, n_k: int,
                  d: int, ldo: int, ldvt: int, scale: float, kv_batch_div: int = 1, accumulate: bool = False,
                  o_scale: float = 1.0, q_batch_mod: int = 0, products: Optional[str] = None, causal: bool = False) -> None:
        f32_products = resolve_f32_products("attention", q.dtype, products, self.f32_products, fused_exact=False)
        self.ensure_init(q.device)
        m = L.AttnMaskArgs()
        a = m.attn
        a.q, a.k, a.vt, a.o = _p(q), _p(k), _p(vt), _p(o)
        a.batch, a.heads, a.n_q, a.n_k, a.d, a.ldo, a.ldvt = batch, heads, n_q, n_k, d, ldo, ldvt
        a.kv_batch_div, a.o_accumulate, a.scale, a.o_scale, a.dtype = kv_batch_div, int(accumulate), scale, o_scale, _dt(q)
        a.q_batch_mod, a.f32_products = q_batch_mod, f32_products
        if not causal:
            self._call("fyc_attention", a)
            return
        m.causal = 1
        self._call("fyc_attention_masked", m)

    def attention_q_batch_mod_supported(self) -> bool:
        return True

    def attention_causal_supported(self) -> bool:
        return self.abi_version >= 308

    def attention_max_head_dim(self) -> int:
        return 512 if self.abi_version >= 308 else 160

    def repeat(self, src: Tensor, dst: Tensor, *, times: int) -> None:
        self.ensure_init(src.device)
        nbytes = src.numel() * src.element_size()
        if src.dtype != dst.dtype or dst.numel() != times * src.numel() or not (src.is_contiguous() and dst.is_contiguous()):
            raise ValueError("repeat: dst must be a contiguous tensor of src's dtype holding `times` copies of src")
        a = L.RepeatArgs()
        a.src, a.dst, a.bytes, a.times = src.data_ptr(), dst.data_ptr(), nbytes, times
        self._call("fyc_repeat", a)

    def temporal_attention(self, qkv: Tensor, o: Tensor, *, clips: int, frames: int, pixels: int, heads: int, d: int,
                           scale: float, rope: Optional[Tuple[Tensor, Tensor]] = None, products: Optional[str] = None) -> None:
        f32_products = resolve_f32_products("temporal_attention", qkv.dtype, products, self.f32_products)
        self.ensure_init(qkv.device)
        a = L.TAttnArgs()
        a.qkv, a.o, a.clips, a.frames, a.pixels, a.heads, a.d, a.scale, a.dtype = (_p(qkv), _p(o), clips, frames, pixels,
                                                                                  heads, d, scale, _dt(qkv))
        if rope is not None:
            cos, sin = rope
            for t in (cos, sin):
                if t.dtype != torch.float32 or not t.is_contiguous() or t.device != qkv.device or tuple(t.shape) != (frames, d // 2):
                    raise ValueError(f"temporal_attention: rope tables must be contiguous f32 [{frames}][{d // 2}] tensors on {qkv.device}")
            a.rope_cos, a.rope_sin = cos.data_ptr(), sin.data_ptr()
        a.f32_products = f32_products
        self._call("fyc_temporal_attention", a)

    def _tblock_args(self, x, out, w_qkv, colsum, bias, pe_bias, w_out, b_out, clips, frames, pixels, heads, d, scale, eps):
# ... 293 lines not shown
```

### followyourclick_amd/profiling.py

```python
from __future__ import annotations

from collections import defaultdict
from typing import Dict

import torch


def _esize(t) -> int:
    return t.element_size()


class TimedOps:
    def __init__(self, inner):
        self.inner = inner
        self.name = inner.name
        self.records = []
        self.enabled = True

    def ensure_init(self, device):
        return self.inner.ensure_init(device)

    def set_tuning(self, key, value):
        return self.inner.set_tuning(key, value)

    def device_caps(self):
        return self.inner.device_caps()

    def _timed(self, family: str, flops: float, nbytes: float, fn, *a, _key=None, **kw):
        if not self.enabled:
            return fn(*a, **kw)
        s, e = torch.cuda.Event(enable_timing=True), torch.cuda.Event(enable_timing=True)
        s.record()
        r = fn(*a, **kw)
        e.record()
        self.records.append((family, s, e, flops, nbytes, _key))
        return r

    def gemm(self, a, w, out, **kw):
        M, N, K, batch = kw["M"], kw["N"], kw["K"], kw.get("batch", 1)
        flops = 2.0 * M * N * K * batch
        es = _esize(a)
        mode = kw.get("mode", 0)
        if mode == 0:
            in_bytes = M * K * es * batch
            fam = "gemm"
        else:
            c = kw["conv"]
            frames = M // (c["Hout"] * c["Wout"])
            in_bytes = frames * c["Hin"] * c["Win"] * c["Cin"] * es
            fam = "conv3x3"
        out_cols = N // 2 if kw.get("epilogue", 0) == 1 else N
        nbytes = in_bytes + N * K * es * batch + M * out_cols * es * batch
        if kw.get("residual") is not None:
            nbytes += M * N * es
        key = f"{fam} M={M} N={N} K={K} b={batch} epi={kw.get('epilogue', 0)} res={int(kw.get('residual') is not None)}"
        return self._timed(fam, flops, nbytes, self.inner.gemm, a, w, out, _key=key, **kw)

    def attention(self, q, k, vt, o, **kw):
        B, H, nq, nk, d = kw["batch"], kw["heads"], kw["n_q"], kw["n_k"], kw["d"]
        flops = 4.0 * B * H * nq * nk * d
        kvb = (B + kw.get("kv_batch_div", 1) - 1) // kw.get("kv_batch_div", 1)
        qb = kw.get("q_batch_mod", 0) or B
        nbytes = ((B + qb) * H * nq * d + 2 * kvb * H * nk * d) * 2
        fam = "attn_self" if nq == nk else "attn_cross"
        return self._timed(fam, flops, nbytes, self.inner.attention, q, k, vt, o, _key=f"{fam} B={B} H={H} nq={nq} nk={nk} d={d}", **kw)

    def attention_q_batch_mod_supported(self):
        fn = getattr(self.inner, "attention_q_batch_mod_supported", None)
        return bool(fn and fn())

    def attention_causal_supported(self):
        fn = getattr(self.inner, "attention_causal_supported", None)
        return bool(fn and fn())

    def attention_max_head_dim(self):
        fn = getattr(self.inner, "attention_max_head_dim", None)
        return int(fn()) if fn else 160

    def repeat(self, src, dst, **kw):
        n = src.numel() * src.element_size()
        return self._timed("repeat", 0.0, (1.0 + kw["times"]) * n, self.inner.repeat, src, dst, **kw)

    def temporal_attention(self, qkv, o, **kw):
        n = kw["clips"] * kw["frames"] * kw["pixels"] * kw["heads"] * kw["d"]
        flops = 4.0 * kw["clips"] * kw["pixels"] * kw["heads"] * kw["frames"] ** 2 * kw["d"]
        return self._timed("attn_temporal", flops, 4.0 * n * _esize(qkv), self.inner.temporal_attention, qkv, o, **kw)

    def gn_stats(self, x, stats, **kw):
        return self._timed("gn_stats", 0.0, kw["rows"] * kw["C_"] * _esize(x), self.inner.gn_stats, x, stats, **kw)

    def gn_apply(self, x, stats, g, b, y, **kw):
        return self._timed("gn_apply", 0.0, 2.0 * kw["rows"] * kw["C_"] * _esize(x), self.inner.gn_apply, x, stats, g, b, y, **kw)

    def gn_apply_cs(self, x1, cs1, g, b, y, **kw):
        return self._timed("gn_apply", 0.0, 2.0 * kw["rows"] * (kw["C1"] + kw.get("C2", 0)) * _esize(x1), self.inner.gn_apply_cs, x1, cs1, g, b, y, **kw)

    def gemm_row_parts(self, dtype, **kw):
        return self.inner.gemm_row_parts(dtype, **kw)

    def gemm_stat_layout(self, dtype, **kw):
        return self.inner.gemm_stat_layout(dtype, **kw)

    def gemm_split_bytes(self, dtype, **kw):
        return self.inner.gemm_split_bytes(dtype, **kw)

    def temporal_block_supported(self, dtype, **kw):
        return self.inner.temporal_block_supported(dtype, **kw)

    def temporal_block(self, x, out, **kw):
        rows, C = kw["clips"] * kw["frames"] * kw["pixels"], kw["heads"] * kw["d"]
        return self._timed("temporal_block", 2.0 * rows * C * 4 * C + 4.0 * rows * kw["frames"] * C, 2.0 * rows * C * _esize(x),
                           self.inner.temporal_block, x, out, **kw)

    def ff_block_supported(self, dtype, **kw):
        return self.inner.ff_block_supported(dtype, **kw)

    def ff_block(self, x, residual, out, **kw):
        rows, C, hid = kw["rows"], kw["C_"], kw["hidden"]
        flops = 2.0 * rows * (C * 2 * hid + (C + hid) * C)
        nbytes = (2 + (residual is not None)) * rows * C * _esize(x) + (C * 2 * hid + (C + hid) * C) * _esize(x)
        return self._timed("ff_block", flops, nbytes, self.inner.ff_block, x, residual, out, **kw)

    def panel_linear_supported(self, dtype, **kw):
        return self.inner.panel_linear_supported(dtype, **kw)

    def panel_linear(self, x, out, **kw):
        rows, N, K = kw["rows"], kw["N"], kw["K"]
        nbytes = (rows * K + rows * N * (2 if kw.get("residual") is not None else 1) + N * K) * _esize(x)
        key = f"panel_linear M={rows} N={N} K={K} gn={int(kw.get('gn_cs') is not None)} res={int(kw.get('residual') is not None)}"
        return self._timed("panel_linear", 2.0 * rows * N * K, nbytes, self.inner.panel_linear, x, out, _key=key, **kw)

    def chan_stats_reduce(self, parts, cs, **kw):
        return self._timed("gn_stats", 0.0, 0.0, self.inner.chan_stats_reduce, parts, cs, **kw)

    def layernorm(self, x, g, b, y, **kw):
        return self._timed("layernorm", 0.0, 2.0 * kw["rows"] * kw["C_"] * _esize(x), self.inner.layernorm, x, g, b, y, **kw)

    def softmax_rows(self, x, **kw):
        return self._timed("softmax", 0.0, 2.0 * kw["rows"] * kw["cols"] * _esize(x), self.inner.softmax_rows, x, **kw)
# ... 36 lines not shown
```

### include/fyc.h

```cpp
#ifndef FYC_H
#define FYC_H
#include <stddef.h>
#include <stdint.h>

#ifdef __cplusplus
extern "C" {
#endif

#define FYC_VERSION 308

typedef enum { FYC_F32 = 0, FYC_BF16 = 1, FYC_F16 = 2 } fyc_dtype;

int fyc_version(void);
const char* fyc_last_error(void);
int fyc_init(const void* zero_page);
int fyc_device_caps(int64_t* caps);
int fyc_set_tuning(int key, int value);

enum { FYC_GEMM_PLAIN = 0, FYC_GEMM_CONV3X3 = 1, FYC_GEMM_CONV3X3_UP2 = 2, FYC_GEMM_CONV_T3 = 3 };
enum { FYC_EPI_LINEAR = 0, FYC_EPI_GEGLU = 1, FYC_EPI_HEADS = 2 };
enum { FYC_ACT_NONE = 0, FYC_ACT_GELU = 1, FYC_ACT_QUICK_GELU = 2 };
enum { FYC_PRODUCTS_EXACT = 0, FYC_PRODUCTS_SPLIT_BF16 = 1 };

typedef struct {
  const void* a;
  const void* a2;
  const void* w;
  const float* bias;
  const float* rowbias;
  const void* residual;
  void* out;
  void* seg_out[3];
  int32_t seg_transposed[3];
  int32_t seg_ld[3];
  int32_t M, N, K;
  int32_t lda, ldw, ldo, ldr;
  int32_t ldrb;
  int32_t k_split, lda2;
  int64_t stride_a, stride_w, stride_o;
  int32_t batch;
  int32_t mode;
  int32_t epilogue;
  int32_t Hout, Wout, Hin, Win, Cin, conv_stride;
  int32_t conv_pad;
  int32_t rows_per_batch;
  int32_t seg_cols, heads, tokens;
  float out_scale;
  int32_t dtype;
  int32_t tile;
  int32_t act;
  const float* ln_stats;
  const float* ln_colsum;
  int32_t ln_nparts; float ln_eps;
  float* chan_parts; int32_t cs_rows;
  float* row_parts; int32_t row_nparts;
  void* workspace; int64_t workspace_bytes;
  int32_t t3_frames, t3_rows;
  int32_t f32_products;
} fyc_gemm_args;
int fyc_gemm(const fyc_gemm_args* a, void* stream);
int64_t fyc_gemm_workspace_bytes(const fyc_gemm_args* a);
int fyc_gemm_row_parts(const fyc_gemm_args* a);
int fyc_gemm_stat_layout(const fyc_gemm_args* a, int32_t* tile_rows, int32_t* slots);

typedef struct { const float* parts; double* cs; int32_t rows, N, cs_rows, tile_rows, slots, out_rows; } fyc_chan_stats_reduce_args;
int fyc_chan_stats_reduce(const fyc_chan_stats_reduce_args* a, void* stream);

typedef struct {
  const void* q; const void* k; const void* vt; void* o;
  int32_t batch, heads, n_q, n_k, d;
  int32_t ldo;
  int32_t ldvt;
  int32_t kv_batch_div;
  int32_t o_accumulate;
  float scale, o_scale;
  int32_t dtype;
  int32_t q_batch_mod;
  int32_t f32_products;
} fyc_attn_args;
int fyc_attention(const fyc_attn_args* a, void* stream);
typedef struct { fyc_attn_args attn; int32_t causal; } fyc_attn_mask_args;
int fyc_attention_masked(const fyc_attn_mask_args* a, void* stream);

typedef struct {
  const void* qkv; void* o;
  int32_t clips, frames, pixels, heads, d;
  float scale;
  int32_t dtype;
  const float* rope_cos; const float* rope_sin;
  int32_t f32_products;
} fyc_tattn_args;
int fyc_temporal_attention(const fyc_tattn_args* a, void* stream);

typedef struct {
  const void* x; double* stats;
  int32_t rows, C, groups, rows_per_sample;
  int32_t dtype;
  int32_t pad_;
  float* workspace; int64_t workspace_bytes;
} fyc_gn_stats_args;
int fyc_gn_stats(const fyc_gn_stats_args* a, void* stream);
int64_t fyc_gn_stats_workspace(const fyc_gn_stats_args* a);

typedef struct {
  const void* x; const double* stats; const float* gamma; const float* beta; void* y;
  int32_t rows, C, groups, rows_per_sample;
  float eps; int32_t silu;
  int32_t dtype;
} fyc_gn_apply_args;
int fyc_gn_apply(const fyc_gn_apply_args* a, void* stream);

typedef struct {
  const void* x1; const double* cs1; const void* x2; const double* cs2;
  const float* gamma; const float* beta; void* y;
  int32_t C1, C2, rows, groups, rows_per_sample;
  float eps; int32_t silu;
  int32_t dtype;
  int32_t cs_rows;
  const float* parts1; const float* parts2;
  int32_t tile_rows1, slots1, tile_rows2, slots2, parts_cs_rows;
} fyc_gn_apply_cs_args;
int fyc_gn_apply_cs(const fyc_gn_apply_cs_args* a, void* stream);

typedef struct {
  const void* x; const float* gamma; const float* beta; const float* pe; void* y;
  int32_t rows, C; float eps;
  int32_t pe_div, pe_rows;
  int32_t dtype;
} fyc_layernorm_args;
int fyc_layernorm(const fyc_layernorm_args* a, void* stream);

typedef struct { const void* x; float* stats; int32_t rows, C; float eps; int32_t dtype; } fyc_row_stats_args;
int fyc_row_stats(const fyc_row_stats_args* a, void* stream);

typedef struct { void* x; int64_t rows; int32_t cols, ld; int32_t dtype; int32_t causal_rows; } fyc_softmax_args;
int fyc_softmax_rows(const fyc_softmax_args* a, void* stream);

typedef struct { const void* a; const void* b; void* y; int64_t rows; int32_t c1, c2; int32_t dtype; } fyc_concat_args;
int fyc_concat_channels(const fyc_concat_args* a, void* stream);

typedef struct { const void* src; void* dst; int64_t bytes; int32_t times; } fyc_repeat_args;
int fyc_repeat(const fyc_repeat_args* a, void* stream);

typedef struct { const float* x; float* y; int64_t n; } fyc_silu_args;
int fyc_silu_f32(const fyc_silu_args* a, void* stream);

typedef struct { const float* x; void* y; int64_t rows; int32_t cols, ld; int32_t dtype; } fyc_cast_args;
// ... 98 lines not shown
```

Measured before the change: 13.46 frames/s.

## Compute 2x upsample conv as four 2x2 sub-pixel phase convolutions

Adds a phase-decomposed kernel for nearest-2x-upsample followed by 3x3 conv: weights are pre-summed into four 2x2 phase filters and each output phase is computed as a GEMM over the low-resolution input with scattered output rows. This removes the redundant 9-tap reads of duplicated pixels and cuts the conv math to 4 taps per output. It adds a new GEMM mode with output-row remapping and extra packed weights, and only applies to 16-bit dtypes with shapes whose row tiles divide the frame size.

New measurement: 13.73 frames/s (median of 6 runs). +2.0%, better.

```diff
diff --git a/followyourclick_amd/_build.py b/followyourclick_amd/_build.py
--- a/followyourclick_amd/_build.py
+++ b/followyourclick_amd/_build.py
@@ -10,7 +10,7 @@
 EXTRA = os.environ.get("FYC_BUILD_EXTRA", "").split()
 LIB = os.path.abspath(os.environ.get("FYC_BUILD_LIB") or os.path.join(HERE, "libfyc_hip.so"))
 OBJ = os.path.join(HERE, "_obj") if not (EXTRA or os.environ.get("FYC_BUILD_LIB")) else LIB + ".obj"
-SOURCES = ["api.hip", "gemm.hip", "gemm_bf16_plain.hip", "gemm_bf16_conv.hip", "gemm_bf16_act.hip", "gemm_f16_plain.hip", "gemm_f16_conv.hip", "gemm_f16_act.hip", "gemm_f32.hip", "gemm_bf16_t3.hip", "gemm_f16_t3.hip", "gemm_f32_t3.hip", "gemm_f32x3.hip", "gemm_f32x3_t3.hip", "attention.hip", "attention_small.hip", "attention_medium.hip", "attention_large.hip", "attention_small_f16.hip", "attention_medium_f16.hip", "attention_large_f16.hip", "attention_f32x3.hip", "attention_wide.hip", "attention_wide_f16.hip", "attention_wide_f32x3.hip", "temporal_attn.hip", "temporal_attn_f32x3.hip", "temporal_block.hip", "temporal_block_rr.hip", "ff_block.hip", "panel_linear.hip", "norm.hip", "elementwise.hip"]
+SOURCES = ["api.hip", "gemm.hip", "gemm_bf16_plain.hip", "gemm_bf16_conv.hip", "gemm_bf16_act.hip", "gemm_f16_plain.hip", "gemm_f16_conv.hip", "gemm_f16_act.hip", "gemm_f32.hip", "gemm_bf16_t3.hip", "gemm_f16_t3.hip", "gemm_f32_t3.hip", "gemm_f32x3.hip", "gemm_f32x3_t3.hip", "conv_up_phases.hip", "gemm_bf16_up.hip", "gemm_f16_up.hip", "attention.hip", "attention_small.hip", "attention_medium.hip", "attention_large.hip", "attention_small_f16.hip", "attention_medium_f16.hip", "attention_large_f16.hip", "attention_f32x3.hip", "attention_wide.hip", "attention_wide_f16.hip", "attention_wide_f32x3.hip", "temporal_attn.hip", "temporal_attn_f32x3.hip", "temporal_block.hip", "temporal_block_rr.hip", "ff_block.hip", "panel_linear.hip", "norm.hip", "elementwise.hip"]
 FLAGS = ["--offload-arch=gfx950", "-O3", "-std=c++17", "-fPIC", "-ffp-contract=off", "-Wno-unused-value",
          "-mllvm", "-amdgpu-mfma-vgpr-form=1"]
 AGPR_SOURCES = {"ff_block.hip", "panel_linear.hip", "temporal_block_rr.hip", "attention_wide.hip", "attention_wide_f16.hip", "attention_wide_f32x3.hip"}
diff --git a/followyourclick_amd/_lib.py b/followyourclick_amd/_lib.py
--- a/followyourclick_amd/_lib.py
+++ b/followyourclick_amd/_lib.py
@@ -40,6 +40,10 @@
     _fields_ = [("attn", AttnArgs), ("causal", i32)]
 
 
+class ConvUpPhasesArgs(C.Structure):
+    _fields_ = [("gemm", GemmArgs), ("group_rows", i32)]
+
+
 class TAttnArgs(C.Structure):
     _fields_ = [("qkv", vp), ("o", vp), ("clips", i32), ("frames", i32), ("pixels", i32), ("heads", i32), ("d", i32),
                 ("scale", f32), ("dtype", i32), ("rope_cos", vp), ("rope_sin", vp), ("f32_products", i32)]
@@ -173,10 +177,11 @@
     "fyc_gn_apply_cs": GnApplyCsArgs, "fyc_chan_stats_reduce": ChanStatsReduceArgs,
     "fyc_pack_conv3x3": PackConv3x3Args, "fyc_pack_geglu": PackGegluArgs, "fyc_temporal_block": TemporalBlockArgs,
     "fyc_ff_block": FFBlockArgs, "fyc_panel_linear": PanelLinearArgs, "fyc_repeat": RepeatArgs,
+    "fyc_conv_up_phases": ConvUpPhasesArgs,
 }
 MISC = ["fyc_version", "fyc_last_error", "fyc_init", "fyc_device_caps", "fyc_set_tuning", "fyc_gemm_row_parts", "fyc_gemm_stat_layout", "fyc_gemm_workspace_bytes", "fyc_gn_stats_workspace", "fyc_temporal_block_supported", "fyc_temporal_block_wstream_bytes",
         "fyc_ff_block_supported", "fyc_ff_block_wstream_bytes", "fyc_panel_linear_supported", "fyc_panel_linear_wstream_bytes",
-        "fyc_cfg_ddim_rescale_workspace_bytes", "fyc_cfg_solver_workspace_bytes"]
+        "fyc_cfg_ddim_rescale_workspace_bytes", "fyc_cfg_solver_workspace_bytes", "fyc_conv_up_phases_stat_layout", "fyc_conv_up_phases_supported"]
 
 _lib = None
 FYC_VERSION = 308
@@ -235,6 +240,11 @@
     if not ab_build or hasattr(lib, "fyc_cfg_solver_workspace_bytes"):
         lib.fyc_cfg_solver_workspace_bytes.argtypes = [C.POINTER(CfgSolverArgs)]
         lib.fyc_cfg_solver_workspace_bytes.restype = i64
+    if not ab_build or hasattr(lib, "fyc_conv_up_phases_supported"):
+        lib.fyc_conv_up_phases_supported.argtypes = [i32] * 7
+        lib.fyc_conv_up_phases_supported.restype = C.c_int
+        lib.fyc_conv_up_phases_stat_layout.argtypes = [C.POINTER(ConvUpPhasesArgs), C.POINTER(i32), C.POINTER(i32)]
+        lib.fyc_conv_up_phases_stat_layout.restype = C.c_int
     for name, st in OPS.items():
         if ab_build and not hasattr(lib, name):
             continue
diff --git a/followyourclick_amd/csrc/conv_up_phases.hip b/followyourclick_amd/csrc/conv_up_phases.hip
--- /dev/null
+++ b/followyourclick_amd/csrc/conv_up_phases.hip
@@ -0,0 +1,93 @@
+#include "gemm_plan.h"
+
+using namespace fycg;
+
+namespace {
+struct UpPlan { int cfg, ns, bm, colc, wide, row_tiles; };
+
+bool up_plan(const fyc_conv_up_phases_args* u, UpPlan& up) {
+  char unused[512];
+  fyc_gemm_args g = u->gemm;
+  g.mode = FYC_GEMM_CONV3X3; g.epilogue = FYC_EPI_LINEAR; g.act = FYC_ACT_NONE; g.batch = 1;
+  g.cs_rows = u->group_rows;
+  GemmPlan pl;
+  if (g.M <= 0 || g.N <= 0 || u->group_rows <= 0 || !plan_gemm(&g, GEMM_STATS_CHAN, true, pl, unused)) return false;
+  if ((pl.splitk > 1 || u->group_rows % pl.bm != 0) && g.tile == 0) {
+    g.tile = (g.N % 320 == 0) ? 6 : (g.N % 128 == 0 || g.N > 512) ? 1 : 2;
+    if (!plan_gemm(&g, GEMM_STATS_CHAN, true, pl, unused)) return false;
+  }
+  if (pl.splitk > 1 || u->group_rows % pl.bm != 0 || pl.cs_slots != 1 || pl.family != GEMM_FAM_CONV) return false;
+  up.cfg = pl.cfg; up.ns = pl.ns; up.bm = pl.bm; up.colc = pl.colc; up.wide = pl.wide; up.row_tiles = pl.row_tiles;
+  return true;
+}
+
+const char* up_shape_refusal(const fyc_conv_up_phases_args* u) {
+  const fyc_gemm_args* a = &u->gemm;
+  if (!gemm_is16(a->dtype)) return "16-bit dtypes only (FYC_F32 keeps FYC_GEMM_CONV3X3_UP2)";
+  if (a->Cin <= 0 || a->Cin % 64 != 0) return "Cin must be a positive multiple of 64";
+  if (a->N <= 0 || a->N % 8 != 0) return "N (Cout) must be a positive multiple of 8";
+  if (a->Hin <= 0 || a->Win <= 0 || a->Win > 4096) return "Hin / Win must be positive, Win <= 4096";
+  if (a->Hout != 2 * a->Hin || a->Wout != 2 * a->Win) return "the output must be exactly twice the input (other sizes keep FYC_GEMM_CONV3X3_UP2)";
+  const long long hw = (long long)a->Hin * a->Win;
+  if (u->group_rows <= 0 || u->group_rows % hw != 0) return "group_rows must be a whole number of input frames (Hin * Win rows each)";
+  if (a->M <= 0 || a->M % 4 != 0 || (a->M / 4) % u->group_rows != 0) return "M must be 4 * group_rows * (number of groups)";
+  if ((long long)(a->M / 4) * a->Cin >= 0xffffffffll || 4ll * a->N * a->Cin * 4 >= 0xffffffffll) return "an operand has 2^32 elements or more: split the call";
+  return nullptr;
+}
+}
+
+extern "C" int fyc_conv_up_phases_supported(int32_t dtype, int32_t Cin, int32_t Cout, int32_t Hin, int32_t Win, int32_t group_rows, int32_t exact2) {
+  if (!exact2 || group_rows <= 0 || group_rows > (1 << 28)) return 0;
+  fyc_conv_up_phases_args u;
+  memset(&u, 0, sizeof(u));
+  u.gemm.dtype = dtype; u.gemm.Cin = Cin; u.gemm.N = Cout; u.gemm.K = 4 * Cin; u.gemm.ldw = 4 * Cin; u.gemm.ldo = Cout;
+  u.gemm.Hin = Hin; u.gemm.Win = Win; u.gemm.Hout = 2 * Hin; u.gemm.Wout = 2 * Win;
+  u.gemm.M = 4 * group_rows;
+  u.group_rows = group_rows;
+  UpPlan up;
+  return up_shape_refusal(&u) == nullptr && up_plan(&u, up) && up.wide ? 1 : 0;
+}
+
+extern "C" int fyc_conv_up_phases_stat_layout(const fyc_conv_up_phases_args* u, int32_t* tile_rows, int32_t* slots) {
+  UpPlan up;
+  if (u == nullptr || up_shape_refusal(u) != nullptr || !up_plan(u, up)) return 0;
+  if (tile_rows) *tile_rows = up.bm;
+  if (slots) *slots = 1;
+  return up.row_tiles;
+}
+
+extern "C" int fyc_conv_up_phases(const fyc_conv_up_phases_args* u, void* stream) {
+  FYC_REQUIRE(u != nullptr, "fyc_conv_up_phases: null args");
+  const fyc_gemm_args* a = &u->gemm;
+  FYC_REQUIRE(g_fyc_zero_page != nullptr, "fyc_conv_up_phases: fyc_init() not called");
+  FYC_REQUIRE(a->mode == FYC_GEMM_CONV3X3_UP2 && a->epilogue == FYC_EPI_LINEAR && a->act == FYC_ACT_NONE && a->batch <= 1 && a->tile >= 0,
+              "fyc_conv_up_phases: the embedded arguments describe a FYC_GEMM_CONV3X3_UP2 problem with the LINEAR epilogue (mode %d, epilogue %d, act %d, batch %d)",
+              a->mode, a->epilogue, a->act, a->batch);
+  FYC_REQUIRE(a->residual == nullptr && a->rowbias == nullptr && a->a2 == nullptr && a->ln_stats == nullptr && a->ln_colsum == nullptr && a->row_parts == nullptr,
+              "fyc_conv_up_phases: bias and chan_parts only - residual, rowbias, a2, a folded LayerNorm and row_parts are not built for the phase form");
+  const char* why = up_shape_refusal(u);
+  FYC_REQUIRE(why == nullptr, "fyc_conv_up_phases: %s (M=%d N=%d Cin=%d Hin=%d Win=%d Hout=%d Wout=%d group_rows=%d dtype=%d)", why, a->M, a->N, a->Cin, a->Hin,
+              a->Win, a->Hout, a->Wout, u->group_rows, a->dtype);
+  FYC_REQUIRE(a->K == 4 * a->Cin && a->ldw >= a->K && a->ldw % 8 == 0, "fyc_conv_up_phases: K=%d must be 4*Cin and ldw=%d a multiple of 8 >= K (weights [4 phases][N][ldw])", a->K, a->ldw);
+  FYC_REQUIRE(4ll * a->N * a->ldw < 0xffffffffll, "fyc_conv_up_phases: the phase weights have 2^32 elements or more");
+  FYC_REQUIRE(a->a != nullptr && a->w != nullptr && a->out != nullptr && ((uintptr_t)a->a % 16) == 0 && ((uintptr_t)a->w % 16) == 0, "fyc_conv_up_phases: a / w / out must be set, a and w 16-byte aligned");
+  FYC_REQUIRE(a->chan_parts == nullptr || (a->cs_rows == u->group_rows && ((uintptr_t)a->chan_parts % 8) == 0),
+              "fyc_conv_up_phases: chan_parts are per (group, phase): cs_rows=%d must equal group_rows=%d (8-byte aligned)", a->cs_rows, u->group_rows);
+  UpPlan up;
+  FYC_REQUIRE(up_plan(u, up), "fyc_conv_up_phases: no row tile divides group_rows=%d (a multiple of 128 is needed; N=%d): keep FYC_GEMM_CONV3X3_UP2", u->group_rows, a->N);
+  FYC_REQUIRE(up.wide, "fyc_conv_up_phases: the 16-byte epilogue needs ldo=%d a multiple of 8 and 16-byte aligned out / bias", a->ldo);
+  GemmP p;
+  memset(&p, 0, sizeof(p));
+  p.a = (const char*)a->a; p.w = (const char*)a->w; p.bias = a->bias; p.out = (char*)a->out;
+  p.M = a->M; p.N = a->N; p.K = a->K; p.lda = a->Cin; p.ldw = a->ldw; p.ldo = a->ldo; p.ldr = a->ldo;
+  p.mode = GEMM_MODE_UP_PHASES; p.epilogue = FYC_EPI_LINEAR;
+  p.Hout = a->Hout; p.Wout = a->Wout; p.Hin = a->Hin; p.Win = a->Win; p.Cin = a->Cin; p.conv_stride = 1; p.conv_pad = 1;
+  p.rows_per_batch = 1; p.ldrb = a->N;
+  p.out_scale = a->out_scale;
+  p.chan_parts = a->chan_parts; p.cs_rows = u->group_rows; p.cs_slots = 1;
+  p.t3_rows = u->group_rows;
+  p.up_sw = 1.0f / (float)a->Win;
+  p.wide = 1; p.colc = up.colc;
+  p.zero = (const char*)g_fyc_zero_page;
+  return a->dtype == FYC_F16 ? run_f16_up_phases(p, up.cfg, up.ns, (hipStream_t)stream) : run_bf16_up_phases(p, up.cfg, up.ns, (hipStream_t)stream);
+}
diff --git a/followyourclick_amd/csrc/gemm_bf16_up.hip b/followyourclick_amd/csrc/gemm_bf16_up.hip
--- /dev/null
+++ b/followyourclick_amd/csrc/gemm_bf16_up.hip
@@ -0,0 +1,6 @@
+#include "gemm_kernel.h"
+namespace fycg {
+int run_bf16_up_phases(const GemmP& p, int cfg, int ns, hipStream_t st) {
+  return dispatch_cfg<bf16_t, GEMM_MODE_UP_PHASES, FYC_EPI_LINEAR, true>(cfg, ns, p, 1, st);
+}
+}
diff --git a/followyourclick_amd/csrc/gemm_f16_up.hip b/followyourclick_amd/csrc/gemm_f16_up.hip
--- /dev/null
+++ b/followyourclick_amd/csrc/gemm_f16_up.hip
@@ -0,0 +1,6 @@
+#include "gemm_kernel.h"
+namespace fycg {
+int run_f16_up_phases(const GemmP& p, int cfg, int ns, hipStream_t st) {
+  return dispatch_cfg<f16_t, GEMM_MODE_UP_PHASES, FYC_EPI_LINEAR, true>(cfg, ns, p, 1, st);
+}
+}
diff --git a/followyourclick_amd/csrc/gemm_kernel.h b/followyourclick_amd/csrc/gemm_kernel.h
--- a/followyourclick_amd/csrc/gemm_kernel.h
+++ b/followyourclick_amd/csrc/gemm_kernel.h
@@ -7,6 +7,8 @@
 namespace fycg {
 
 constexpr int FYC_MAX_DEVICES = 64;
+
+constexpr int GEMM_MODE_UP_PHASES = 16;
 
 struct GemmP {
   const char* a; const char* a2; const char* w; const float* bias; const float* rowbias; const char* residual; char* out;
@@ -368,6 +370,13 @@
   const int n_lane = n_w0 + lch * 8;
   const int first_sample = do_cs ? (tile_m * BM) / p.cs_rows : 0;
   const bool one_slot = p.cs_slots == 1;
+  int up_xb = 0, up_o0 = 0;
+  if constexpr (MODE == GEMM_MODE_UP_PHASES) {
+    const int m0 = tile_m * BM, vs = m0 / p.t3_rows, phase = vs & 3;
+    const int q0 = (vs >> 2) * p.t3_rows + (m0 - vs * p.t3_rows);
+    up_xb = q0 % p.Win;
+    up_o0 = 4 * q0 + 2 * (phase >> 1) * p.Win + (phase & 1);
+  }
   float cs8[8], cq8[8];
 #pragma unroll
   for (int e = 0; e < 8; ++e) cs8[e] = cq8[e] = 0.f;
@@ -417,9 +426,14 @@
       const int m = tile_m * BM + (wm * WTM + i) * 16 + row;
       float rsum = 0.f, rsq = 0.f;
       const bool live = lact && row < 16 && m < p.M && n_lane < p.N;
+      int mo = m;
+      if constexpr (MODE == GEMM_MODE_UP_PHASES) {
+        const int d = (wm * WTM + i) * 16 + row, xd = up_xb + d;
+        mo = up_o0 + 4 * d - 2 * (xd - fdiv_small(xd, p.up_sw) * p.Win);
+      }
       if (live) {
         const u32x4 v4 = v4q;
-        *reinterpret_cast<u32x4*>(O + (long long)m * p.ldo + n_lane) = v4;
+        *reinterpret_cast<u32x4*>(O + (long long)mo * p.ldo + n_lane) = v4;
         if (do_cs || do_rp) {
 #pragma unroll
           for (int e = 0; e < 4; ++e) {
@@ -700,6 +714,7 @@
                                               long long bz, char* stg_stage, int wave, int lane, const char* pre, int& ecnt) {
   constexpr int WTM = BM / WGM / 16, WTN = BN / WGN / 16;
   constexpr bool LN = (MODE == FYC_GEMM_PLAIN);
+  static_assert(MODE != GEMM_MODE_UP_PHASES || (WIDE && EPI == FYC_EPI_LINEAR && sizeof(T) == 2), "UP_PHASES: the packed 16-bit LINEAR epilogue only");
   const int wm = wave / WGN, wn = wave % WGN;
   const int g = lane >> 4, r16 = lane & 15;
   T* O = reinterpret_cast<T*>(p.out) + bz * p.stride_o;
@@ -1106,9 +1121,10 @@
   static_assert(ROWS_IT % 16 == 0, "row stride per DMA instruction must keep the swizzle key");
   int i_tm = 0, i_tn = 0;
   unsigned a_base = 0, a2_base = 0, b_base = 0;
-  constexpr bool C3 = (MODE == FYC_GEMM_CONV3X3);
+  constexpr bool UPP = (MODE == GEMM_MODE_UP_PHASES);
+  constexpr bool C3 = (MODE == FYC_GEMM_CONV3X3) || UPP;
   constexpr bool T3 = (MODE == FYC_GEMM_CONV_T3);
-  constexpr int TAPS = T3 ? 3 : 9;
+  constexpr int TAPS = T3 ? 3 : UPP ? 4 : 9;
   static_assert(!T3 || A_IT * 3 <= 32, "CONV_T3: the presence masks of a thread's rows share one register");
   int a_pos[C3 ? A_IT : 1], a_msk[C3 ? A_IT : 1];
   unsigned t_msk = 0, t_step = 0;
@@ -1139,6 +1155,25 @@
         const unsigned msk = (f > 0 ? 1u : 0u) | 2u | (f + 1 < p.t3_frames ? 4u : 0u);
         if (m < p.M) t_msk |= msk << (3 * it);
       }
+    } else if constexpr (UPP) {
+      const int m0 = i_tm * BM, vs = m0 / p.t3_rows, phase = vs & 3;
+      const int q0 = (vs >> 2) * p.t3_rows + (m0 - vs * p.t3_rows);
+      b_base += (unsigned)phase * (unsigned)p.N * (unsigned)p.ldw;
+      const int hw = p.Hin * p.Win;
+#pragma unroll
+      for (int it = 0; it < A_IT; ++it) {
+        const int q = q0 + lrow + it * ROWS_IT;
+        const int fr = q / hw, rem = q - fr * hw, y = rem / p.Win, x = rem - y * p.Win;
+        const int iy0 = y - 1 + (phase >> 1), ix0 = x - 1 + (phase & 1);
+        a_pos[it] = fr * hw + iy0 * p.Win + ix0;
+        int msk = 0;
+#pragma unroll
+        for (int tp = 0; tp < 4; ++tp) {
+          const int iy = iy0 + (tp >> 1), ix = ix0 + (tp & 1);
+          if ((unsigned)iy < (unsigned)p.Hin && (unsigned)ix < (unsigned)p.Win) msk |= 1 << tp;
+        }
+        a_msk[it] = (m0 + lrow + it * ROWS_IT < p.M) ? msk : 0;
+      }
     } else {
 #pragma unroll
       for (int it = 0; it < A_IT; ++it) {
@@ -1174,7 +1209,7 @@
       const unsigned e = a_base + (unsigned)(it * ROWS_IT) * (unsigned)p.Cin + (unsigned)(tap - 1) * t_step + (unsigned)c0;
       return ((t_msk >> (3 * it + tap)) & 1u) ? A + (size_t)e : zero;
     } else if (C3) {
-      const int ky = tap / 3, kx = tap - 3 * ky;
+      const int ky = UPP ? tap >> 1 : tap / 3, kx = UPP ? tap & 1 : tap - 3 * ky;
       const int pos = a_pos[it] + ky * p.Win + kx;
       return ((a_msk[it] >> tap) & 1) ? A + (size_t)((unsigned)pos * (unsigned)p.Cin + (c0 + koff)) : zero;
     } else {
@@ -1541,5 +1576,7 @@
 int run_bf16_t3(const GemmP& p, int batch, int cfg, int ns, hipStream_t st);
 int run_f16_t3(const GemmP& p, int batch, int cfg, int ns, hipStream_t st);
 int run_f32_t3(const GemmP& p, int batch, int cfg, hipStream_t st);
-
-}
+int run_bf16_up_phases(const GemmP& p, int cfg, int ns, hipStream_t st);
+int run_f16_up_phases(const GemmP& p, int cfg, int ns, hipStream_t st);
+
+}
diff --git a/followyourclick_amd/engine/base.py b/followyourclick_amd/engine/base.py
--- a/followyourclick_amd/engine/base.py
+++ b/followyourclick_amd/engine/base.py
@@ -127,12 +127,34 @@
                              eps=eps, silu=silu, **kw)
         return y
 
+    def _up_phases_group(self, w: Tensor, w_ph: Optional[Tensor], frames: int, Hin: int, Win: int, Ho: int, Wo: int, out_rows: int) -> int:
+        supported = getattr(self.ops, "conv_up_phases_supported", None)
+        if (w_ph is None or supported is None or os.environ.get("FYC_UP_PHASES", "1") == "0" or self.dtype not in (torch.bfloat16, torch.float16)
+                or (Ho, Wo) != (2 * Hin, 2 * Win)):
+            return 0
+        G = out_rows // 4 if out_rows else Hin * Win
+        if G <= 0 or G % (Hin * Win) or (frames * Hin * Win) % G:
+            return 0
+        Cout, K = w.shape
+        return G if supported(self.dtype, Cin=K // 9, Cout=Cout, Hin=Hin, Win=Win, group_rows=G, exact2=True) else 0
+
     def conv_stats(self, x: Tensor, w: Tensor, b: Tensor, frames: int, Hin: int, Win: int, nxt=None, per_frame: bool = False,
-                   stride: int = 1, pad: int = 1, up2: bool = False, up_size=None, **kw) -> Tuple[Tensor, Optional[ChanStats]]:
+                   stride: int = 1, pad: int = 1, up2: bool = False, up_size=None, w_ph: Optional[Tensor] = None, **kw) -> Tuple[Tensor, Optional[ChanStats]]:
         Cout, K = w.shape
         Ho, Wo = conv_out_size(Hin, Win, stride, pad, up2, up_size)
         if per_frame:
             nxt = (Ho * Wo, Ho * Wo)
+        G = self._up_phases_group(w, w_ph, frames, Hin, Win, Ho, Wo, nxt[1] if nxt is not None else 0) if up2 and not kw else 0
+        if G:
+            st = None
+            if nxt is not None and self.fuse_stats:
+                nt, tile_rows, slots = self.ops.conv_up_phases_stat_layout(self.dtype, frames=frames, Hin=Hin, Win=Win, Cin=K // 9, Cout=Cout, group_rows=G)
+                st = ChanStats(Cout, 4 * G, parts=self.new(nt * slots * Cout * 2, dtype=torch.float32), tile_rows=tile_rows, slots=slots,
+                               rows=frames * Ho * Wo, stat_rows=G)
+            out = self.new(frames * Ho * Wo, Cout)
+            self.ops.conv_up_phases(x, w_ph, out, frames=frames, Hin=Hin, Win=Win, Cin=K // 9, Cout=Cout, group_rows=G, bias=b,
+                                    chan_parts=None if st is None else st.parts)
+            return out, self._produced(st)
         st = None
         if nxt is not None:
             st = self._cs_plan(frames * Ho * Wo, nxt[0], Cout, K, L.GEMM_CONV3X3_UP2 if up2 else L.GEMM_CONV3X3, nxt[1])
diff --git a/followyourclick_amd/engine/unet3d.py b/followyourclick_amd/engine/unet3d.py
--- a/followyourclick_amd/engine/unet3d.py
+++ b/followyourclick_amd/engine/unet3d.py
@@ -492,7 +492,7 @@
                 Hn, Wn = sizes[-1]
                 g2 = dict(g, H=Hn, W=Wn)
                 g2["rows"] = B * F * Hn * Wn
-                x = self._conv_act(x.t, blk.up.w, blk.up.b, frames, g["H"], g["W"], clip(g2), up2=True, up_size=(Hn, Wn))
+                x = self._conv_act(x.t, blk.up.w, blk.up.b, frames, g["H"], g["W"], clip(g2), up2=True, up_size=(Hn, Wn), w_ph=blk.up.get("w_ph"))
                 g = g2
         h, _ = self._gn(x, P.out_g, P.out_b, g["rows"], clip(g)[1], cfg.norm_eps, True)
         return self.conv(h, P.conv_out_w, P.conv_out_b, frames, g["H"], g["W"])
diff --git a/followyourclick_amd/engine/vae.py b/followyourclick_amd/engine/vae.py
--- a/followyourclick_amd/engine/vae.py
+++ b/followyourclick_amd/engine/vae.py
@@ -79,7 +79,7 @@
             for r in blk.resnets:
                 x, cs = self.resnet(r, x, N, H, W, cs)
             if blk.up is not None:
-                x, cs = self.conv_cs(x, blk.up.w, blk.up.b, N, H, W, up2=True)
+                x, cs = self.conv_cs(x, blk.up.w, blk.up.b, N, H, W, up2=True, w_ph=blk.up.get("w_ph"))
                 H, W = 2 * H, 2 * W
         c0 = cfg.block_out_channels[0]
         h = self.gn(x, cs, P.out_g, P.out_b, N * H * W, c0, H * W, True)
diff --git a/followyourclick_amd/engine/weights.py b/followyourclick_amd/engine/weights.py
--- a/followyourclick_amd/engine/weights.py
+++ b/followyourclick_amd/engine/weights.py
@@ -28,6 +28,34 @@
     p[:, :I] = w
     p = p.reshape(O, Ip // sl, sl, 3, 3).permute(0, 1, 3, 4, 2)
     return p.reshape(O, 9 * Ip).to(dtype).contiguous().to(device)
+
+
+def up_phase_weights(w: Tensor) -> Tensor:
+    rows = ((w[:, :, 0], w[:, :, 1] + w[:, :, 2]), (w[:, :, 0] + w[:, :, 1], w[:, :, 2]))
+    out = []
+    for py in range(2):
+        for px in range(2):
+            taps = []
+            for ty in range(2):
+                r = rows[py][ty]
+                cols = ((r[..., 0], r[..., 1] + r[..., 2]), (r[..., 0] + r[..., 1], r[..., 2]))[px]
+                taps.append(torch.stack(cols, dim=-1))
+            out.append(torch.stack(taps, dim=-2))
+    return torch.stack(out, dim=0)
+
+
+def pack_conv_up_phases(w: Tensor, dtype, device) -> Tensor:
+    O, I, kh, kw = w.shape
+    assert kh == 3 and kw == 3
+    Ip, sl = pad_channels(I), conv_slab(dtype)
+    p = torch.zeros(4, O, Ip, 2, 2, dtype=torch.float32)
+    p[:, :, :I] = up_phase_weights(w.detach().float())
+    p = p.reshape(4, O, Ip // sl, sl, 2, 2).permute(0, 1, 2, 4, 5, 3)
+    return p.reshape(4, O, 4 * Ip).to(dtype).contiguous().to(device)
+
+
+def _up_phases(w: Tensor, dtype, device) -> Optional[Tensor]:
+    return pack_conv_up_phases(w, dtype, device) if dtype in (torch.bfloat16, torch.float16) else None
 
 
 def pack_conv_t3(w: Tensor, dtype, device) -> Tensor:
@@ -381,7 +409,8 @@
                 if cfg.use_motion_module and (2 ** (nb - 1 - i)) in cfg.motion_module_resolutions else None))
         us = None
         if i != nb - 1:
-            us = Packed(w=pack_conv3x3(sd[f"{p}.upsamplers.0.conv.weight"], dtype, device), b=f32(sd[f"{p}.upsamplers.0.conv.bias"], device))
+            us = Packed(w=pack_conv3x3(sd[f"{p}.upsamplers.0.conv.weight"], dtype, device), b=f32(sd[f"{p}.upsamplers.0.conv.bias"], device),
+                        w_ph=_up_phases(sd[f"{p}.upsamplers.0.conv.weight"], dtype, device))
         up.append(Packed(layers=layers, up=us))
     P["up"] = up
     P["out_g"], P["out_b"] = f32(sd["conv_norm_out.weight"], device), f32(sd["conv_norm_out.bias"], device)
@@ -414,7 +443,7 @@
         us = None
         if i != nb - 1:
             k = f"decoder.up_blocks.{i}.upsamplers.0.conv"
-            us = Packed(w=pack_conv3x3(sd[k + ".weight"], dtype, device), b=f32(sd[k + ".bias"], device))
+            us = Packed(w=pack_conv3x3(sd[k + ".weight"], dtype, device), b=f32(sd[k + ".bias"], device), w_ph=_up_phases(sd[k + ".weight"], dtype, device))
         ups.append(Packed(resnets=rs, up=us))
     P["ups"] = ups
     P["out_g"], P["out_b"] = f32(sd["decoder.conv_norm_out.weight"], device), f32(sd["decoder.conv_norm_out.bias"], device)
diff --git a/followyourclick_amd/ops.py b/followyourclick_amd/ops.py
--- a/followyourclick_amd/ops.py
+++ b/followyourclick_amd/ops.py
@@ -186,6 +186,44 @@
         a.parts, a.cs, a.rows, a.N, a.cs_rows, a.tile_rows, a.slots = _f32(parts, "parts"), _p(cs), rows, N, cs_rows, tile_rows, slots
         a.out_rows = out_rows
         self._call("fyc_chan_stats_reduce", a)
+
+    def conv_up_phases_supported(self, dtype: torch.dtype, *, Cin: int, Cout: int, Hin: int, Win: int, group_rows: int, exact2: bool = True) -> bool:
+        if not hasattr(self.lib, "fyc_conv_up_phases_supported") or dtype not in (torch.bfloat16, torch.float16):
+            return False
+        key = ("cups", dtype, Cin, Cout, Hin, Win, group_rows, bool(exact2))
+        if key not in self._q_cache:
+            self._q_cache[key] = bool(self.lib.fyc_conv_up_phases_supported(_dtc(dtype), Cin, Cout, Hin, Win, group_rows, int(bool(exact2))))
+        return self._q_cache[key]
+
+    @staticmethod
+    def _conv_up_phases_args(dtype_code: int, frames: int, Hin: int, Win: int, Cin: int, Cout: int, ldw: int, ldo: int, group_rows: int):
+        u = L.ConvUpPhasesArgs()
+        g = u.gemm
+        g.M, g.N, g.K, g.lda, g.ldw, g.ldo = 4 * frames * Hin * Win, Cout, 4 * Cin, Cin, ldw, ldo
+        g.mode, g.epilogue, g.batch, g.out_scale, g.dtype = L.GEMM_CONV3X3_UP2, L.EPI_LINEAR, 1, 1.0, dtype_code
+        g.Hout, g.Wout, g.Hin, g.Win, g.Cin, g.conv_stride, g.conv_pad = 2 * Hin, 2 * Win, Hin, Win, Cin, 1, 1
+        u.group_rows = group_rows
+        return u
+
+    def conv_up_phases_stat_layout(self, dtype: torch.dtype, *, frames: int, Hin: int, Win: int, Cin: int, Cout: int, group_rows: int):
+        key = ("cupl", dtype, frames, Hin, Win, Cin, Cout, group_rows)
+        if key not in self._q_cache:
+            u = self._conv_up_phases_args(_dtc(dtype), frames, Hin, Win, Cin, Cout, 4 * Cin, Cout, group_rows)
+            tr, sl = L.i32(0), L.i32(0)
+            n = int(self.lib.fyc_conv_up_phases_stat_layout(C.byref(u), C.byref(tr), C.byref(sl)))
+            self._q_cache[key] = (n, int(tr.value), int(sl.value))
+        return self._q_cache[key]
+
+    def conv_up_phases(self, x: Tensor, w_ph: Tensor, out: Tensor, *, frames: int, Hin: int, Win: int, Cin: int, Cout: int, group_rows: int,
+                       bias: Optional[Tensor] = None, ldo: int = 0, chan_parts: Optional[Tensor] = None) -> None:
+        self.ensure_init(x.device)
+        if x.dtype != w_ph.dtype:
+            raise TypeError(f"conv_up_phases: activation {x.dtype} vs weight {w_ph.dtype}")
+        u = self._conv_up_phases_args(_dt(x), frames, Hin, Win, Cin, Cout, w_ph.shape[-1], ldo or Cout, group_rows)
+        g = u.gemm
+        g.a, g.w, g.bias, g.out = _p(x), _p(w_ph), _f32(bias, "bias"), _p(out)
+        g.chan_parts, g.cs_rows = _f32(chan_parts, "chan_parts"), (group_rows if chan_parts is not None else 0)
+        self._call("fyc_conv_up_phases", u)
 
     @staticmethod
     def _gemm_args(a, w, out, *, M, N, K, lda, ldw, ldo, bias, rowbias, rows_per_batch, residual, ldr, ldrb, out_scale, epilogue, mode,
diff --git a/followyourclick_amd/profiling.py b/followyourclick_amd/profiling.py
--- a/followyourclick_amd/profiling.py
+++ b/followyourclick_amd/profiling.py
@@ -55,6 +55,20 @@
             nbytes += M * N * es
         key = f"{fam} M={M} N={N} K={K} b={batch} epi={kw.get('epilogue', 0)} res={int(kw.get('residual') is not None)}"
         return self._timed(fam, flops, nbytes, self.inner.gemm, a, w, out, _key=key, **kw)
+
+    def conv_up_phases_supported(self, dtype, **kw):
+        fn = getattr(self.inner, "conv_up_phases_supported", None)
+        return bool(fn and fn(dtype, **kw))
+
+    def conv_up_phases_stat_layout(self, dtype, **kw):
+        return self.inner.conv_up_phases_stat_layout(dtype, **kw)
+
+    def conv_up_phases(self, x, w_ph, out, **kw):
+        M, N, K = 4 * kw["frames"] * kw["Hin"] * kw["Win"], kw["Cout"], 4 * kw["Cin"]
+        es = _esize(x)
+        nbytes = (M // 4 * kw["Cin"] + 4 * N * K + M * N) * es
+        key = f"conv3x3 up_phases M={M} N={N} K={K} b=1 epi=0 res=0"
+        return self._timed("conv3x3", 2.0 * M * N * K, nbytes, self.inner.conv_up_phases, x, w_ph, out, _key=key, **kw)
 
     def attention(self, q, k, vt, o, **kw):
         B, H, nq, nk, d = kw["batch"], kw["heads"], kw["n_q"], kw["n_k"], kw["d"]
diff --git a/include/fyc.h b/include/fyc.h
--- a/include/fyc.h
+++ b/include/fyc.h
@@ -63,6 +63,11 @@
 int fyc_gemm_row_parts(const fyc_gemm_args* a);
 int fyc_gemm_stat_layout(const fyc_gemm_args* a, int32_t* tile_rows, int32_t* slots);
 
+typedef struct { fyc_gemm_args gemm; int32_t group_rows; } fyc_conv_up_phases_args;
+int fyc_conv_up_phases(const fyc_conv_up_phases_args* a, void* stream);
+int fyc_conv_up_phases_stat_layout(const fyc_conv_up_phases_args* a, int32_t* tile_rows, int32_t* slots);
+int fyc_conv_up_phases_supported(int32_t dtype, int32_t Cin, int32_t Cout, int32_t Hin, int32_t Win, int32_t group_rows, int32_t exact2);
+
 typedef struct { const float* parts; double* cs; int32_t rows, N, cs_rows, tile_rows, slots, out_rows; } fyc_chan_stats_reduce_args;
 int fyc_chan_stats_reduce(const fyc_chan_stats_reduce_args* a, void* stream);
 
```
